# OPENAIRINTERFACE/openairinterface5g

Measured on AMD Instinct MI355X. Metric: ldpc_decoder_coded_throughput, higher is better.
Workload: dtype int8

## Files before the change

openairinterface5g_amd/csrc/ldpc_dec_fast_block.h:

```cpp
#ifndef LDPC_DEC_FAST_BLOCK_H
#define LDPC_DEC_FAST_BLOCK_H
#include <hip/hip_runtime.h>
#include "ldpc_kernels.h"
#include "ldpc_dec_fast_core.h"

typedef const ldpc_dec_job LDPC_CONST_AS *ldpc_job_ptr_t;


#ifndef LDPC_DEC_LLR_ARGS
#define LDPC_DEC_LLR_ARGS 1
#endif
#ifndef LDPC_DEC_LLR_TOGETHER
#define LDPC_DEC_LLR_TOGETHER 1
#endif
#ifndef LDPC_DEC_WARM
#define LDPC_DEC_WARM 0
#endif

#ifndef LDPC_MUTE_ITEMS
#define LDPC_MUTE_ITEMS 1
#endif
#define LDPC_EAGER_MAX_BAD_LANES 96
#define LDPC_TIMING_SLOTS 28
#ifndef LDPC_SYN_SKIP
#define LDPC_SYN_SKIP 1
#endif

#define LDPC_Q_TICKET(w) ((int)((uint32_t)(w) & 0xffffu))
#define LDPC_Q_BAD(w) ((int)((uint32_t)(w) >> 16))

__device__ __forceinline__ int ldpc_draw(int *counter, int lane)
{
  int t = 0;
  if (lane == 0)
    t = atomicAdd(counter, 1);
  return LDPC_UNIFORM(t);
}

__device__ __forceinline__ int ldpc_draw_count(int *counter, int lane, uint32_t syn)
{
  const int cnt = (int)__popcll(__ballot(syn != 0));
  int t = 0;
  if (lane == 0)
    t = atomicAdd(counter, 1 + (cnt << 16));
  return LDPC_UNIFORM(t);
}

__device__ __forceinline__ int ldpc_draw_issue(int *counter, int lane)
{
  int t = 0;
  if (lane == 0)
    t = __hip_atomic_fetch_add(counter, 1, __ATOMIC_RELAXED, __HIP_MEMORY_SCOPE_WORKGROUP);
  return t;
}

__device__ __forceinline__ int ldpc_desc_n_app(ldpc_code_ptr_t code, int zq) { return code->ncore * zq; }
__device__ __forceinline__ int ldpc_desc_n_ext(ldpc_code_ptr_t code, int zq) { return code->f_ext_global ? 0 : (code->ncols - code->ncore) * zq; }

#if defined(__HIP_DEVICE_COMPILE__)
#define LDPC_STAMP_BEHIND_S(x) asm volatile("" ::"s"(x) : "memory")
#define LDPC_STAMP_BEHIND_V(x) asm volatile("" ::"v"(x) : "memory")
#define LDPC_STAMP_BEHIND_ALL() __builtin_amdgcn_s_waitcnt(0)
#else
#define LDPC_STAMP_BEHIND_S(x) do { volatile uint32_t ldpc_keep_ = (uint32_t)(x); (void)ldpc_keep_; } while (0)
#define LDPC_STAMP_BEHIND_V(x) LDPC_STAMP_BEHIND_S(x)
#define LDPC_STAMP_BEHIND_ALL() ((void)0)
#endif

__device__ __forceinline__ void ldpc_fast_tables_to_lds(uint8_t *fsm, ldpc_code_ptr_t code, int tid, int nt)
{
  const uint32_t lds0 = ldpc_lds_addr(fsm);
  const int ext_global = code->f_ext_global, ncore = code->ncore, nedges = code->nedges, Z = code->Z;
  uint32_t *etbl = reinterpret_cast<uint32_t *>(fsm + code->f_lds_etbl);
  uint32_t *ctbl = reinterpret_cast<uint32_t *>(fsm + code->f_lds_ctbl);
  uint32_t *rowtbl = reinterpret_cast<uint32_t *>(fsm + code->f_lds_rowtbl);
  uint32_t *coltbl = reinterpret_cast<uint32_t *>(fsm + code->f_lds_coltbl);
  for (int i = tid; i < nedges; i += nt)
    etbl[i] = code->f_etbl[i] + ((ext_global && code->e_col[i] >= ncore) ? 0u : lds0);
  for (int i = tid; i < 2 * code->f_n_ctbl; i += nt)
    ctbl[i] = code->f_ctbl[i] + ((i & 1) ? lds0 : 0u);
  for (int i = tid; i < code->nrows; i += nt)
    rowtbl[i] = code->f_rowtbl[i];
  for (int i = tid; i < ncore; i += nt)
    coltbl[i] = code->f_coltbl[i];
  for (int i = tid; i < (Z + 4) >> 2; i += nt)
    reinterpret_cast<uint32_t *>(fsm + code->f_lds_zero)[i] = 0u;
}

__device__ __forceinline__ bool ldpc_fast_item_is_mute(const ldpc_fast_lds &L, int e0, int deg, int j)
{
  const uint32_t info = L.etbl[e0 + deg - 1];
  const uint32_t lw = L.ext_global ? (*reinterpret_cast<const uint32_t *>(L.gllr + info + 4u * (uint32_t)j) ^ 0x80808080u)
                                   : ldpc_lds_ld32(L.base, info + 4u * (uint32_t)j);
  return lw == 0x80808080u;
}
__device__ __forceinline__ void ldpc_fast_item_zero_messages(const ldpc_fast_lds &L, int e0, int deg, int j, int Z, int rstride)
{
  uint8_t *rrow = L.r + e0 * rstride + 4 * j;
  uint8_t *rpad = rrow + (j == 0 ? Z : 0);
  for (int k = 0; k < deg; k++) {
    *reinterpret_cast<uint32_t *>(rrow + k * rstride) = 0x80808080u;
    *reinterpret_cast<uint32_t *>(rpad + k * rstride) = 0x80808080u;
  }
}

template <class IO, int ZC = 0>
__device__ __forceinline__ int ldpc_dec_fast_block(uint8_t *fsm, ldpc_code_ptr_t code, const IO &io)
{
  const int Z = ZC ? ZC : code->Z, zq = ZC ? ZC / 4 : code->f_zq, rstride = ZC ? ZC + 4 : code->f_rstride,
            astride = ZC ? 2 * ZC : code->f_astride;
  const uint32_t zq_magic = ZC ? (uint32_t)((0x100000000ULL + (unsigned long long)(ZC ? ZC / 4 : 1) - 1) / (unsigned long long)(ZC ? ZC / 4 : 1))
                               : code->f_zq_magic;
  const uint32_t z_magic = 0xffffffffu / (uint32_t)Z + 1u;
  ldpc_fast_lds L;
  L.base = fsm;
  L.r = fsm + code->f_lds_r;
  L.app = fsm + code->f_lds_app;
  L.ext = fsm + code->f_lds_ext;
  uint32_t *etbl = reinterpret_cast<uint32_t *>(fsm + code->f_lds_etbl);
  uint32_t *ctbl = reinterpret_cast<uint32_t *>(fsm + code->f_lds_ctbl);
  uint32_t *rowtbl = reinterpret_cast<uint32_t *>(fsm + code->f_lds_rowtbl);
  uint32_t *coltbl = reinterpret_cast<uint32_t *>(fsm + code->f_lds_coltbl);
  L.etbl = etbl; L.ctbl = ctbl; L.rowtbl = rowtbl; L.coltbl = coltbl;
  int *flags = reinterpret_cast<int *>(fsm + code->f_lds_misc);
  const int tid = io.tid(), nt = blockDim.x, lane = tid & 63;
  const int ncore = code->ncore, num_llr = code->num_llr, ncz = ncore * Z;
  const uint32_t *__restrict__ src32 = io.src32();
  const uint32_t *__restrict__ srcp = io.src32_prologue();
  uint32_t *stage = io.stage_core();

  const int ext_global = code->f_ext_global;
  L.gllr = reinterpret_cast<const uint8_t *>(src32);
  L.ext_global = ext_global;
  const int n_app = io.n_app(code, zq), n_ext = io.n_ext(code, zq);
  uint32_t va[4], ve[4];
  if (!stage) {
#pragma unroll
    for (int k = 0; k < 4; k++) {
      const int ia = tid + k * nt;
#if LDPC_DEC_LLR_TOGETHER
      va[k] = io.ld_llr(srcp + (ia < n_app ? ia : 0));
      ve[k] = io.ld_llr(srcp + (ia < n_ext ? n_app + ia : 0));
#else
      va[k] = ia < n_app ? io.ld_llr(srcp + ia) : 0u;
      ve[k] = ia < n_ext ? io.ld_llr(srcp + n_app + ia) : 0u;
#endif
    }
  }
  if constexpr (IO::pass_stamps) {
    if (tid == 0) {
      LDPC_STAMP_BEHIND_S(ncore + num_llr + ext_global);
      io.stamps()[42] = (uint32_t)wall_clock64();
    }
    if (tid == nt - 64) {
      LDPC_STAMP_BEHIND_V(va[0]);
      io.stamps()[43] = (uint32_t)wall_clock64();
    }
  }
  const bool have_tables = io.tables_resident();
  if (!have_tables)
    ldpc_fast_tables_to_lds(fsm, code, tid, nt);
  if constexpr (IO::pass_stamps) {
    if (tid == 0) {
      LDPC_STAMP_BEHIND_ALL();
      io.stamps()[44] = (uint32_t)wall_clock64();
    }
  }
  if (stage) {
#pragma unroll
    for (int k = 0; k < 4; k++) {
      const int ia = tid + k * nt;
      va[k] = ia < n_app ? io.ld_llr(srcp + ia) : 0u;
      ve[k] = ia < n_ext ? io.ld_llr(srcp + n_app + ia) : 0u;
    }
  }
  if (tid < 16)
    flags[tid] = 0;
  uint32_t *e32 = reinterpret_cast<uint32_t *>(L.ext);
#pragma unroll
  for (int k = 0; k < 4; k++) {
    const int i = tid + k * nt;
    if (i < n_app) {
      const int c = (int)ldpc_umulhi((uint32_t)i, zq_magic), j = i - c * zq;
      const uint32_t w = va[k] ^ 0x80808080u;
      uint32_t *dst = reinterpret_cast<uint32_t *>(L.app + c * astride) + j;
      dst[0] = w;
      dst[zq] = w;
      if (stage)
        stage[i] = va[k];
    }
    if (i < n_ext)
      e32[i] = ve[k] ^ 0x80808080u;
  }
  for (int i = tid + 4 * nt; i < n_app; i += nt) {
    const int c = (int)ldpc_umulhi((uint32_t)i, zq_magic), j = i - c * zq;
    const uint32_t v = io.ld_llr(srcp + i), w = v ^ 0x80808080u;
    uint32_t *dst = reinterpret_cast<uint32_t *>(L.app + c * astride) + j;
    dst[0] = w;
    dst[zq] = w;
    if (stage)
      stage[i] = v;
  }
  for (int i = tid + 4 * nt; i < n_ext; i += nt)
    e32[i] = io.ld_llr(srcp + n_app + i) ^ 0x80808080u;
  __syncthreads();
  if (io.stamps() && tid == 0)
    io.stamps()[0] = (uint32_t)wall_clock64();

  const int max_pass = io.max_pass();
  int n_iter = max_pass;
  const int n_cn_tasks = code->f_n_cn_tasks, n_bn_tickets = code->f_n_bn_tickets, n_bn_tasks = code->f_n_bn_tasks,
            bn_group = code->f_bn_group;
  int cn_ticket = 0;
  bool mute_check = false;
  if constexpr (!IO::syndrome && IO::mute_items)
    mute_check = io.mute_check();
  (void)mute_check;
#ifdef LDPC_TIMING
  long long *tlog = reinterpret_cast<long long *>(io.out()) + (tid >> 6) * 2 * LDPC_TIMING_SLOTS;
  int tlog_n = 0;
  const long long t_kernel0 = clock64();
#define LDPC_TLOG_BEGIN() const long long tl0_ = clock64()
#define LDPC_TLOG_END(phase, deg) \
  do { \
    if (blockIdx.x == 0 && p == 2 && lane == 0 && tlog_n < LDPC_TIMING_SLOTS) { \
      tlog[2 * tlog_n] = ((tl0_ - t_kernel0) << 20) | ((long long)(phase) << 8) | (long long)(deg); \
      tlog[2 * tlog_n + 1] = clock64() - t_kernel0; \
      tlog_n++; \
    } \
  } while (0)
#define LDPC_TSTAMP(id) \
  do { \
    LDPC_TLOG_BEGIN(); \
    LDPC_TLOG_END(3, id); \
  } while (0)
#else
#define LDPC_TLOG_BEGIN() do { } while (0)
#define LDPC_TLOG_END(phase, deg) do { } while (0)
#define LDPC_TSTAMP(id) do { } while (0)
#endif
  const int fair = io.fair_turns();
  int prio_slot = 0;
  if (fair)
    prio_slot = (int)(__builtin_amdgcn_s_getreg((3 << 11) | 4) & 15u) / fair;
  for (int p = 1; p <= max_pass; ++p) {
    uint32_t tsyn = 0;
    bool skip = false;
    if (fair) {
      if ((p + prio_slot) & 1)
        __builtin_amdgcn_s_setprio(1);
      else
        __builtin_amdgcn_s_setprio(0);
    }
    if constexpr (IO::warm_next && LDPC_DEC_WARM != 0) {
      if (p == 2 && tid >= nt - 64) {
        if (const uint32_t *nx = io.warm_row()) {
          const int n_lines = (num_llr + 127) >> 7, last = (num_llr >> 2) - 1;
          uint32_t got = 0;
          for (int t0 = lane; t0 <= n_lines; t0 += 256) {
#pragma unroll
            for (int k = 0; k < 4; k++) {
              const int i = 32 * (t0 + 64 * k);
              got ^= nx[i < last ? i : last];
            }
          }
          LDPC_STAMP_BEHIND_V(got);
        }
      }
    }
    const uint32_t ab_word = (io.has_abort() && tid == 0 && p >= 2) ? io.abort_load() : 0u;
    int tb_ab = 0;
    if (io.has_abort() && tid == 0 && p >= 2 && io.tb_abort())
      tb_ab = __hip_atomic_load(io.tb_abort(), __ATOMIC_RELAXED, __HIP_MEMORY_SCOPE_AGENT);
    int *const pq = &flags[8 + (p & 1)];
#ifdef LDPC_ABLATE_CN
    int task = cn_ticket;
    if (IO::syndrome && lane == 0)
      atomicAdd(pq, 64 << 16);
#else
    if (p == 1)
      cn_ticket = LDPC_Q_TICKET(ldpc_draw(pq, lane));
    int task = cn_ticket;
    auto next_task = [&]() -> int {
      if constexpr (IO::syndrome) {
        const int w = ldpc_draw_count(pq, lane, tsyn);
        skip = LDPC_SYN_SKIP && LDPC_Q_BAD(w) > LDPC_EAGER_MAX_BAD_LANES;
        if constexpr (IO::pass_stamps) {
          if (skip && LDPC_Q_TICKET(w) < n_cn_tasks && lane == 0)
            atomicAdd(&flags[7], 1);
        }
        return LDPC_Q_TICKET(w);
      } else {
        return LDPC_Q_TICKET(ldpc_draw(pq, lane));
      }
    };
    for (; task < n_cn_tasks; task = next_task()) {
      LDPC_TLOG_BEGIN();
      tsyn = 0;
      bool with_syn = false;
      if constexpr (IO::syndrome)
        with_syn = p >= 2 && !skip;
      const int deg_f = code->f_cn_task[task][0], ext = code->f_cn_task[task][1];
      const int item = code->f_cn_task[task][2] + lane;
      const int gstart = code->f_cn_task[task][3], gend = code->f_cn_task[task][4], srow0 = code->f_cn_task[task][5];
      const int deg = deg_f & 0xff;
      if (deg_f & 0x100) {
        if (item < gend) {
          const int item_b = item + 64 < gend ? item + 64 : item;
          const int gia = item - gstart, gib = item_b - gstart;
          const int riga = (int)ldpc_umulhi((uint32_t)gia, zq_magic), ja = gia - riga * zq;
          const int rigb = (int)ldpc_umulhi((uint32_t)gib, zq_magic), jb = gib - rigb * zq;
          const uint32_t reca = rowtbl[srow0 + riga], recb = rowtbl[srow0 + rigb];
          const int e0a = (int)(reca & 0x1ffu), e0b = (int)(recb & 0x1ffu);
          uint32_t mb = 0;
          bool mute = false;
          if constexpr (!IO::syndrome && IO::mute_items)
            mute = mute_check && ldpc_fast_item_is_mute(L, e0a, deg, ja) && ldpc_fast_item_is_mute(L, e0b, deg, jb);
          if (mute) {
            if (p == 1) {
              ldpc_fast_item_zero_messages(L, e0a, deg, ja, Z, rstride);
              ldpc_fast_item_zero_messages(L, e0b, deg, jb, Z, rstride);
            }
          } else if (p == 1)
            (void)ldpc_fast_cn2_dispatch<true, false>(deg, L, e0a, ja, e0b, jb, Z, rstride, mb);
          else if (with_syn) {
            if constexpr (IO::syndrome) {
              const uint32_t ma = ldpc_fast_cn2_dispatch<false, true>(deg, L, e0a, ja, e0b, jb, Z, rstride, mb);
              const int valida = (int)(reca >> 16) - 4 * ja, validb = (int)(recb >> 16) - 4 * jb;
              tsyn = (ma & ldpc_fast_valid_lanes(valida)) | (mb & ldpc_fast_valid_lanes(validb));
            }
          } else
            (void)ldpc_fast_cn2_dispatch<false, false>(deg, L, e0a, ja, e0b, jb, Z, rstride, mb);
        }
      } else if (item < gend) {
        const bool pair = deg == 19 && code->f_pair19;
        const int gi = pair ? (item - gstart) >> 1 : item - gstart, half = (item - gstart) & 1;
        const int rig = (int)ldpc_umulhi((uint32_t)gi, zq_magic), j = gi - rig * zq;
        const uint32_t rowrec = rowtbl[srow0 + rig];
        const int e0 = (int)(rowrec & 0x1ffu);
        (void)half;
#if !defined(__HIP_DEVICE_COMPILE__)
        if (pair && half)
          continue;
#endif
        bool mute = false;
        if constexpr (!IO::syndrome && IO::mute_items)
          mute = mute_check && ext && ldpc_fast_item_is_mute(L, e0, deg, j);
        if (mute) {
          if (p == 1)
            ldpc_fast_item_zero_messages(L, e0, deg, j, Z, rstride);
        } else if (p == 1) {
#if defined(__HIP_DEVICE_COMPILE__)
          if (pair)
            (void)ldpc_fast_cn19_pair<true, false>(L, e0, j, Z, rstride, half);
          else
#endif
            (void)ldpc_fast_cn_dispatch<true, false>(deg, ext, L, e0, j, Z, rstride);
        } else if (with_syn) {
          if constexpr (IO::syndrome) {
            uint32_t m;
#if defined(__HIP_DEVICE_COMPILE__)
            if (pair)
              m = ldpc_fast_cn19_pair<false, true>(L, e0, j, Z, rstride, half);
            else
#endif
              m = ldpc_fast_cn_dispatch<false, true>(deg, ext, L, e0, j, Z, rstride);
            const int valid = (int)(rowrec >> 16) - 4 * j;
            tsyn = m & ldpc_fast_valid_lanes(valid);
          }
        } else {
#if defined(__HIP_DEVICE_COMPILE__)
          if (pair)
            (void)ldpc_fast_cn19_pair<false, false>(L, e0, j, Z, rstride, half);
          else
#endif
            (void)ldpc_fast_cn_dispatch<false, false>(deg, ext, L, e0, j, Z, rstride);
        }
      }
      LDPC_TLOG_END(0, deg);
    }
#endif
    const int bn_ticket = task - n_cn_tasks;
    if (tid == 0) {
      flags[2] = 0;
      flags[8 + ((p + 1) & 1)] = 0;
      if (tb_ab)
        flags[3] = 1;
      if (p >= 2 && io.abort_is(ab_word))
        flags[3] = 1;
    }
    __syncthreads();
    const int bad_prev = LDPC_Q_BAD(__hip_atomic_load(pq, __ATOMIC_RELAXED, __HIP_MEMORY_SCOPE_WORKGROUP));
    if constexpr (IO::pass_stamps) {
      if (tid == 0 && p <= 9) {
        io.stamps()[2 * p] = (uint32_t)wall_clock64();
        io.stamps()[22 + p] = (uint32_t)bad_prev;
        io.stamps()[32 + p] = (uint32_t)flags[7];
      }
      if (tid == 0)
        flags[7] = 0;
    }
    if (io.has_abort() && flags[3]) {
      n_iter = max_pass + 1;
      break;
    }
    if (!io.use_crc() && p >= 3 && bad_prev == 0) {
      n_iter = p - 1;
      break;
    }
#ifndef LDPC_ABLATE_BN
    if constexpr (IO::bn_tickets) {
    for (int ticket = bn_ticket, nxt = 0; ticket < n_bn_tickets; ticket = LDPC_Q_TICKET(LDPC_UNIFORM(nxt)) - n_cn_tasks) {
      LDPC_TLOG_BEGIN();
      const int item0 = code->f_bn_rec[ticket][0] + lane, end = code->f_bn_rec[ticket][1];
      const int maxdeg = code->f_bn_rec[ticket][2], cnt = code->f_bn_rec[ticket][3];
      if (cnt == 1) {
        if (item0 < end) {
          const int sc = (int)ldpc_umulhi((uint32_t)item0, zq_magic), j = item0 - sc * zq;
          const uint32_t colrec = coltbl[sc];
          const uint32_t lw = src32[(int)(colrec & 0xffu) * zq + j];
          uint32_t ae = 0, at = 0;
          ldpc_fast_bn_gather(L, colrec, maxdeg, j, Z, 0, ae, at);
          nxt = ldpc_draw_issue(pq, lane);
          ldpc_fast_bn_finish(L, (int)(colrec & 0xffu), (int)((colrec >> 8) & 0xffu), j, Z, astride, lw, ae, at, 0);
        } else {
          nxt = ldpc_draw_issue(pq, lane);
        }
      } else {
        uint32_t rec[LDPC_F_BN_GROUP], lw[LDPC_F_BN_GROUP];
        int jj[LDPC_F_BN_GROUP];
        bool live[LDPC_F_BN_GROUP];
#pragma unroll
        for (int g = 0; g < LDPC_F_BN_GROUP; g++) {
          const int item = item0 + 64 * g;
          live[g] = g < cnt && item < end;
          const int it = live[g] ? item : end - 1;
          const int sc = (int)ldpc_umulhi((uint32_t)it, zq_magic);
          jj[g] = it - sc * zq;
          rec[g] = coltbl[sc];
          lw[g] = src32[(int)(rec[g] & 0xffu) * zq + jj[g]];
        }
        ldpc_fast_bn_multi<LDPC_F_BN_GROUP>(L, rec, jj, lw, live, maxdeg, Z, astride);
        nxt = ldpc_draw_issue(pq, lane);
      }
      LDPC_TLOG_END(1, maxdeg);
    }
    } else {
    for (int ticket = bn_ticket; ticket * bn_group < n_bn_tasks; ticket = LDPC_Q_TICKET(ldpc_draw(pq, lane)) - n_cn_tasks) {
      for (int task = ticket * bn_group; task < (ticket + 1) * bn_group && task < n_bn_tasks; task++) {
        LDPC_TLOG_BEGIN();
        const int item = code->f_bn_task[task][0] + lane, end = code->f_bn_task[task][1];
        const int maxdeg = code->f_bn_task[task][2];
        if (item < end) {
          const int sc = (int)ldpc_umulhi((uint32_t)item, zq_magic), j = item - sc * zq;
          const uint32_t colrec = coltbl[sc];
          const uint32_t lw = src32[(int)(colrec & 0xffu) * zq + j];
          ldpc_fast_bn(L, colrec, maxdeg, j, Z, astride, lw);
        }
        LDPC_TLOG_END(1, maxdeg);
      }
    }
    }
#endif
    cn_ticket = LDPC_Q_TICKET(ldpc_draw(&flags[8 + ((p + 1) & 1)], lane));
    __syncthreads();
    if constexpr (IO::pass_stamps) {
      if (tid == 0 && p <= 9)
        io.stamps()[2 * p + 1] = (uint32_t)wall_clock64();
    }
    if (io.eager_check() && !io.use_crc() && p >= 2 && p < max_pass && bad_prev <= LDPC_EAGER_MAX_BAD_LANES) {
      if constexpr (IO::pass_stamps) {
        if (tid == 0)
          io.stamps()[20] |= 1u << p;
      }
      uint32_t esyn = 0;
      const int n_items = code->nrows * zq;
      for (int item = tid; item < n_items; item += nt) {
        const int sr = (int)ldpc_umulhi((uint32_t)item, zq_magic), j = item - sr * zq;
        const uint32_t rowrec = rowtbl[sr];
        const int e0 = (int)(rowrec & 0x1ffu), deg = (int)((rowrec >> 9) & 0x1fu), ext = (int)((rowrec >> 14) & 1u);
        const int valid = (int)(rowrec >> 16) - 4 * j;
        const uint32_t m = ldpc_fast_pc(L, deg, ext, e0, j, rstride);
        esyn |= m & ldpc_fast_valid_lanes(valid);
      }
      if (__any(esyn != 0) && lane == 0)
        flags[6] = 1;
      __syncthreads();
      const int bad = flags[6];
      __syncthreads();
      if (tid == 0)
        flags[6] = 0;
      if (!bad) {
        n_iter = p;
        break;
      }
      __syncthreads();
    }
    if (io.use_crc() && p >= 3) {
      uint32_t x = 0;
      const int crcE = io.crcE();
      const uint32_t *crc_pow = io.crc_pow();
#pragma unroll 1
      for (int i = 4 * tid; i < crcE; i += 4 * nt) {
        const int c = (int)ldpc_umulhi((uint32_t)i, z_magic), u = i - c * Z;
        const uint32_t nb = ~*reinterpret_cast<const uint32_t *>(L.app + c * astride + u);
        const uint4 pw = *reinterpret_cast<const uint4 *>(crc_pow + (crcE - 4 - i));
        const uint32_t p3 = pw.w, p2 = pw.z, p1 = pw.y, p0 = pw.x;
        x ^= (p3 & (0u - ((nb >> 7) & 1u))) ^ (p2 & (0u - ((nb >> 15) & 1u))) ^ (p1 & (0u - ((nb >> 23) & 1u))) ^
             (p0 & (0u - (nb >> 31)));
      }
      for (int off = 32; off; off >>= 1)
        x ^= __shfl_xor(x, off);
      if (lane == 0 && x)
        atomicXor(reinterpret_cast<unsigned int *>(&flags[2]), x);
      __syncthreads();
      const int rem = flags[2];
      __syncthreads();
      if (rem == 0) {
        n_iter = p;
        break;
      }
    }
  }
  if (io.stamps() && tid == 0)
    io.stamps()[1] = (uint32_t)wall_clock64();
  if (io.tb_abort() && n_iter == max_pass && tid == 0)
    __hip_atomic_store(io.tb_abort(), 1, __ATOMIC_RELAXED, __HIP_MEMORY_SCOPE_AGENT);

#ifdef LDPC_TIMING
  if (blockIdx.x == 0)
    return n_iter;
#endif
  auto bits_word = [&](int w) -> uint32_t {
    uint32_t word = 0;
#pragma unroll
    for (int q = 0; q < 8; q++) {
      const int b = 32 * w + 4 * q;
      if (b < ncz) {
        const int c = (int)ldpc_umulhi((uint32_t)b, z_magic), u = b - c * Z;
        const uint32_t nb = ~*reinterpret_cast<const uint32_t *>(L.app + c * astride + u);
        const uint32_t nib = (((nb >> 7) & 1u) << 3) | (((nb >> 15) & 1u) << 2) | (((nb >> 23) & 1u) << 1) | (nb >> 31);
        word |= nib << (8 * (q >> 1) + ((q & 1) ? 0 : 4));
      }
    }
    return word;
  };
  auto bytes_word = [&](int w) -> uint32_t {
    const int b = 4 * w;
    if (b >= ncz)
      return 0u;
    const int c = (int)ldpc_umulhi((uint32_t)b, z_magic), u = b - c * Z;
    const uint32_t nb = ~*reinterpret_cast<const uint32_t *>(L.app + c * astride + u);
    return (nb >> 7) & 0x01010101u;
  };
  if constexpr (IO::tb_epilogue) {
    if (io.tb_fused()) {
      io.tb_finish(n_iter, bits_word, flags);
      return n_iter;
    }
  }
  if ((!io.use_crc() || n_iter >= 3) && n_iter <= max_pass) {
    const uint32_t tag = io.out_tag();
    const int nwords = io.out_mode() == 0 ? (num_llr + 31) >> 5 : num_llr >> 2;
    if (tag) {
      uint4 *o16 = reinterpret_cast<uint4 *>(io.out());
      for (int c = tid; 3 * c < nwords; c += nt) {
        uint32_t w3[3];
#pragma unroll
        for (int q = 0; q < 3; q++) {
          const int w = 3 * c + q;
          w3[q] = w < nwords ? (io.out_mode() == 0 ? bits_word(w) : bytes_word(w)) : 0u;
        }
        io.put16(o16 + c, w3[0], w3[1], w3[2], tag);
      }
    } else if (io.out_mode() == 0) {
      uint32_t *o = reinterpret_cast<uint32_t *>(io.out());
      for (int w = tid; w < nwords; w += nt)
        o[w] = bits_word(w);
    } else {
      int8_t *o = io.out();
      for (int i = tid; i < num_llr; i += nt)
        o[i] = (i < ncz) ? (int8_t)ldpc_fast_hd(L, i, Z, z_magic, astride) : (int8_t)0;
    }
  }
  return n_iter;
}
#endif
```

openairinterface5g_amd/csrc/ldpc_dec_fast_core.h:

```cpp
#ifndef LDPC_DEC_FAST_CORE_H
#define LDPC_DEC_FAST_CORE_H
#include "ldpc_dec_core.h"

#if !defined(__HIPCC__)
struct uint2 { uint32_t x, y; };
#endif
typedef short ldpc_v2i __attribute__((ext_vector_type(2)));
typedef unsigned short ldpc_v2u __attribute__((ext_vector_type(2)));

#if defined(__HIP_DEVICE_COMPILE__)
LDPC_HD uint32_t ldpc_perm(uint32_t s0, uint32_t s1, uint32_t sel) { return __builtin_amdgcn_perm(s0, s1, sel); }
LDPC_HD uint32_t ldpc_alignbyte(uint32_t hi, uint32_t lo, uint32_t sh) { return __builtin_amdgcn_alignbyte(hi, lo, sh); }
LDPC_HD uint32_t ldpc_umulhi(uint32_t a, uint32_t b) { return __umulhi(a, b); }
#else
LDPC_HD uint32_t ldpc_perm(uint32_t s0, uint32_t s1, uint32_t sel)
{
  const uint64_t src = ((uint64_t)s0 << 32) | s1;
  uint32_t r = 0;
  for (int i = 0; i < 4; i++) {
    const uint32_t s = (sel >> (8 * i)) & 0xff;
    const uint32_t b = s <= 7    ? (uint32_t)((src >> (8 * s)) & 0xff)
                       : s <= 11 ? (((src >> (16 * (s - 8) + 15)) & 1) ? 0xffu : 0u)
                                 : (s == 0x0c ? 0u : 0xffu);
    r |= b << (8 * i);
  }
  return r;
}
LDPC_HD uint32_t ldpc_alignbyte(uint32_t hi, uint32_t lo, uint32_t sh)
{
  return (uint32_t)(((((uint64_t)hi) << 32) | lo) >> (8 * (sh & 3)));
}
LDPC_HD uint32_t ldpc_umulhi(uint32_t a, uint32_t b) { return (uint32_t)(((uint64_t)a * b) >> 32); }
#endif

LDPC_HD ldpc_v2i ldpc_as_v2i(uint32_t x) { return __builtin_bit_cast(ldpc_v2i, x); }
LDPC_HD ldpc_v2u ldpc_as_v2u(uint32_t x) { return __builtin_bit_cast(ldpc_v2u, x); }
LDPC_HD uint32_t ldpc_u2u32(ldpc_v2u x) { return __builtin_bit_cast(uint32_t, x); }
LDPC_HD ldpc_v2u ldpc_splatu(unsigned v) { return (ldpc_v2u){(unsigned short)v, (unsigned short)v}; }
LDPC_HD ldpc_v2u ldpc_pminu(ldpc_v2u a, ldpc_v2u b) { return __builtin_elementwise_min(a, b); }
LDPC_HD ldpc_v2u ldpc_pmaxu(ldpc_v2u a, ldpc_v2u b) { return __builtin_elementwise_max(a, b); }
#define LDPC_KEY_NEUTRAL 0xfbffu
LDPC_HD ldpc_v2u ldpc_pmin3_keys(ldpc_v2u a, ldpc_v2u b, ldpc_v2u c)
{
#if defined(__HIP_DEVICE_COMPILE__)
  uint32_t r;
  asm("v_pk_maximum3_f16 %0, %1, %2, %3" : "=v"(r) : "v"(__builtin_bit_cast(uint32_t, a)), "v"(__builtin_bit_cast(uint32_t, b)),
      "v"(__builtin_bit_cast(uint32_t, c)));
  return __builtin_bit_cast(ldpc_v2u, r);
#else
  return __builtin_elementwise_min(__builtin_elementwise_min(a, b), c);
#endif
}
LDPC_HD uint32_t ldpc_psub_sm(uint32_t a, uint32_t r)
{
#if defined(__HIP_DEVICE_COMPILE__)
  typedef _Float16 ldpc_v2h __attribute__((ext_vector_type(2)));
  const uint32_t d = __builtin_bit_cast(uint32_t, __builtin_bit_cast(ldpc_v2h, a) - __builtin_bit_cast(ldpc_v2h, r));
  return d;
#else
  uint32_t d = 0;
  for (int h = 0; h < 32; h += 16) {
    const uint32_t x = (a >> h) & 0xffffu, y = (r >> h) & 0xffffu;
    d |= (x < y ? 0x8000u | (y - x) : x - y) << h;
  }
  return d;
#endif
}
LDPC_HD ldpc_v2u ldpc_sm_key(uint32_t d) { return __builtin_bit_cast(ldpc_v2u, d | 0x80008000u); }
LDPC_HD uint32_t ldpc_unpack_even(uint32_t w) { return w & 0x00ff00ffu; }
LDPC_HD uint32_t ldpc_unpack_odd(uint32_t w) { return ldpc_perm(0u, w, 0x0c030c01u); }
LDPC_HD uint32_t ldpc_as_u32(ldpc_v2i x) { return __builtin_bit_cast(uint32_t, x); }
LDPC_HD ldpc_v2i ldpc_splat(int v) { return (ldpc_v2i){(short)v, (short)v}; }
LDPC_HD ldpc_v2i ldpc_pmin(ldpc_v2i a, ldpc_v2i b) { return __builtin_elementwise_min(a, b); }
LDPC_HD ldpc_v2i ldpc_pmax(ldpc_v2i a, ldpc_v2i b) { return __builtin_elementwise_max(a, b); }
LDPC_HD ldpc_v2i ldpc_unpack_lo(uint32_t w) { return ldpc_as_v2i(ldpc_perm(0u, w, 0x0c010c00u)); }
LDPC_HD ldpc_v2i ldpc_unpack_hi(uint32_t w) { return ldpc_as_v2i(ldpc_perm(0u, w, 0x0c030c02u)); }
LDPC_HD uint32_t ldpc_pack4(ldpc_v2i lo, ldpc_v2i hi) { return ldpc_perm(ldpc_as_u32(hi), ldpc_as_u32(lo), 0x06040200u); }

struct ldpc_fast_lds {
  uint8_t *base;
  uint8_t *r;
  uint8_t *app;
  uint8_t *ext;
  const uint32_t *etbl, *ctbl, *rowtbl, *coltbl;
  const uint8_t *gllr;
  int ext_global;
};

#if defined(__HIP_DEVICE_COMPILE__)
LDPC_HD uint32_t ldpc_lds_addr(const uint8_t *p) { return (uint32_t)(uintptr_t)(const __attribute__((address_space(3))) uint8_t *)p; }
LDPC_HD uint32_t ldpc_lds_ld32(const uint8_t *, uint32_t a) { return *(const __attribute__((address_space(3))) uint32_t *)a; }
#else
LDPC_HD uint32_t ldpc_lds_addr(const uint8_t *) { return 0u; }
LDPC_HD uint32_t ldpc_lds_ld32(const uint8_t *base, uint32_t a) { return *reinterpret_cast<const uint32_t *>(base + a); }
#endif
LDPC_HD uint32_t ldpc_window_al(const uint8_t *base, uint32_t a, uint32_t sh)
{
  return ldpc_alignbyte(ldpc_lds_ld32(base, a + 4u), ldpc_lds_ld32(base, a), sh);
}
LDPC_HD uint32_t ldpc_window(const uint8_t *base, uint32_t off) { return ldpc_window_al(base, off & ~3u, off); }

#define LDPC_SEL_EO 0x07030501u
#define LDPC_SEL_SIGNS 0x0b090a08u
template <uint32_t SEL = 0x07050301u>
LDPC_HD uint32_t ldpc_fast_odd_lanes(uint32_t parw, bool ext, uint32_t extl, uint32_t exth, int D)
{
  uint32_t np = parw >> 7;
  if (ext)
    np ^= ldpc_perm(exth, extl, SEL);
  if (D & 1)
    np = ~np;
  return np & 0x01010101u;
}
LDPC_HD uint32_t ldpc_fast_valid_lanes(int valid) { return valid > 0 ? 0x01010101u : 0u; }
LDPC_HD uint32_t ldpc_fast_cn_sign_acc(uint32_t sx4, uint32_t s4_prev, uint32_t s4_k, int k, int D)
{
  if (k & 1) {
#if defined(__HIP_DEVICE_COMPILE__)
    return __builtin_amdgcn_bitop3_b32(sx4, s4_prev, s4_k, 0x96);
#else
    return sx4 ^ s4_prev ^ s4_k;
#endif
  }
  return k == D - 1 ? sx4 ^ s4_k : sx4;
}
LDPC_HD uint32_t ldpc_fast_cn_out_bytes(uint32_t o4, uint32_t sx4, uint32_t s4)
{
#if defined(__HIP_DEVICE_COMPILE__)
  return __builtin_amdgcn_bitop3_b32(o4, sx4, s4, 0x96) + __builtin_amdgcn_bitop3_b32(sx4, s4, 0x01010101u, 0x28);
#else
  const uint32_t x4 = sx4 ^ s4;
  return (o4 ^ x4) + (x4 & 0x01010101u);
#endif
}

template <bool IS_EXT, bool P1 = false>
LDPC_HD void ldpc_fast_cn_edge(const ldpc_fast_lds &L, uint32_t info, int t, uint32_t rw, bool first, uint32_t &de, uint32_t &dod,
                               uint32_t &parw, uint32_t &exte, uint32_t &exto)
{
  if (IS_EXT) {
    const uint32_t lw = L.ext_global ? (*reinterpret_cast<const uint32_t *>(L.gllr + info + (uint32_t)t) ^ 0x80808080u)
                                     : ldpc_lds_ld32(L.base, info + (uint32_t)t);
    const uint32_t ae = ldpc_unpack_even(lw), ao = ldpc_unpack_odd(lw);
    if (first) {
      exte = ae + (P1 ? 0x00800080u : ldpc_unpack_even(rw));
      exto = ao + (P1 ? 0x00800080u : ldpc_unpack_odd(rw));
    }
    de = ldpc_psub_sm(ae, 0x00800080u);
    dod = ldpc_psub_sm(ao, 0x00800080u);
  } else {
    const uint32_t aw = ldpc_window(L.base, info + (uint32_t)t);
    if (first)
      parw ^= aw;
    if (P1) {
      de = ldpc_psub_sm(ldpc_unpack_even(aw), 0x00800080u);
      dod = ldpc_psub_sm(ldpc_unpack_odd(aw), 0x00800080u);
    } else {
      de = ldpc_psub_sm(ldpc_unpack_even(aw), ldpc_unpack_even(rw));
      dod = ldpc_psub_sm(ldpc_unpack_odd(aw), ldpc_unpack_odd(rw));
    }
  }
}

template <int D, bool EXT, int MODE, bool P1 = false, bool SYN = true>
LDPC_HD uint32_t ldpc_fast_cn(const ldpc_fast_lds &L, int e0, int j, int Z, int rstride, int boff_r = 0, int boff_a = 0)
{
  const int t = 4 * j + boff_r, ta = 4 * j + boff_a;
  constexpr bool KEEP = MODE == 0;
  uint32_t d_lo[MODE <= 1 ? D : 1], d_hi[MODE <= 1 ? D : 1], g_lo[KEEP ? D : 1], g_hi[KEEP ? D : 1];
  ldpc_v2u m1l = ldpc_splatu(0xffff), m2l = m1l, m1h = m1l, m2h = m1l;
  uint32_t sxl = 0, sxh = 0, parw = 0, extl = 0, exth = 0;
  uint8_t *rrow = L.r + e0 * rstride + t;
  uint8_t *rpad = rrow + (j == 0 ? Z : 0);
#pragma unroll
  for (int k = 0; k < D; k++) {
    const uint32_t info = L.etbl[e0 + k];
    const uint32_t rw = (P1 || (!SYN && EXT && k == D - 1)) ? 0u : *reinterpret_cast<const uint32_t *>(rrow + k * rstride);
    uint32_t dl, dh;
    if (EXT && k == D - 1)
      ldpc_fast_cn_edge<true, P1>(L, info, t, rw, SYN, dl, dh, parw, extl, exth);
    else
      ldpc_fast_cn_edge<false, P1>(L, info, ta, rw, SYN, dl, dh, parw, extl, exth);
    if (MODE <= 1) {
      d_lo[k] = dl;
      d_hi[k] = dh;
    }
    const ldpc_v2u ml = ldpc_sm_key(dl);
    const ldpc_v2u mh = ldpc_sm_key(dh);
    if (KEEP) {
      g_lo[k] = ldpc_u2u32(ml);
      g_hi[k] = ldpc_u2u32(mh);
    }
    sxl ^= dl;
    sxh ^= dh;
    m2l = ldpc_pminu(m2l, ldpc_pmaxu(m1l, ml));
    m1l = ldpc_pminu(m1l, ml);
    m2h = ldpc_pminu(m2h, ldpc_pmaxu(m1h, mh));
    m1h = ldpc_pminu(m1h, mh);
  }
  const ldpc_v2u cap = ldpc_splatu(0x8000 + 127);
  m1l = ldpc_pminu(m1l, cap); m2l = ldpc_pminu(m2l, cap);
  m1h = ldpc_pminu(m1h, cap); m2h = ldpc_pminu(m2h, cap);
  const uint32_t sl = (ldpc_u2u32(m1l) - 0x80008000u) + ldpc_u2u32(m2l), sh = (ldpc_u2u32(m1h) - 0x80008000u) + ldpc_u2u32(m2h);
  const uint32_t sx4 = ldpc_perm(sxh, sxl, LDPC_SEL_SIGNS) ^ 0x80808080u;
#pragma unroll
  for (int k = 0; k < D; k++) {
    uint32_t dl, dh;
    if (MODE <= 1) {
      dl = d_lo[k];
      dh = d_hi[k];
    } else {
      const uint32_t info = L.etbl[e0 + k];
      const uint32_t rw = (P1 || (EXT && k == D - 1)) ? 0u : *reinterpret_cast<const uint32_t *>(rrow + k * rstride);
      if (EXT && k == D - 1)
        ldpc_fast_cn_edge<true, P1>(L, info, t, rw, false, dl, dh, parw, extl, exth);
      else
        ldpc_fast_cn_edge<false, P1>(L, info, ta, rw, false, dl, dh, parw, extl, exth);
    }
    const ldpc_v2u ml = KEEP ? ldpc_as_v2u(g_lo[k]) : ldpc_sm_key(dl);
    const ldpc_v2u mh = KEEP ? ldpc_as_v2u(g_hi[k]) : ldpc_sm_key(dh);
    const uint32_t ol = sl - ldpc_u2u32(ldpc_pminu(ml, m2l)), oh = sh - ldpc_u2u32(ldpc_pminu(mh, m2h));
    const uint32_t o4 = ldpc_perm(oh, ol, 0x06020400u);
    const uint32_t w = ldpc_fast_cn_out_bytes(o4, sx4, ldpc_perm(dh, dl, LDPC_SEL_SIGNS));
    *reinterpret_cast<uint32_t *>(rrow + k * rstride) = w;
    *reinterpret_cast<uint32_t *>(rpad + k * rstride) = w;
  }
  return SYN ? ldpc_fast_odd_lanes<LDPC_SEL_EO>(parw, EXT, extl, exth, D) : 0u;
}

template <int D, bool EXT, bool P1 = false, bool SYN = true>
LDPC_HD uint32_t ldpc_fast_cn_ps(const ldpc_fast_lds &L, int e0, int j, int Z, int rstride, int boff_r = 0, int boff_a = 0)
{
  const int t = 4 * j + boff_r, ta = 4 * j + boff_a;
  constexpr int NP = D / 2;
  uint32_t m_lo[D], m_hi[D], p_lo[NP], p_hi[NP], s4[D];
  const ldpc_v2u cap = ldpc_splatu(0x8000 + 127);
  uint32_t sx4 = 0, parw = 0, extl = 0, exth = 0;
  uint8_t *rrow = L.r + e0 * rstride + t;
  uint8_t *rpad = rrow + (j == 0 ? Z : 0);
#pragma unroll
  for (int k = 0; k < D; k++) {
    const uint32_t info = L.etbl[e0 + k];
    const uint32_t rw = (P1 || (!SYN && EXT && k == D - 1)) ? 0u : *reinterpret_cast<const uint32_t *>(rrow + k * rstride);
    uint32_t dl, dh;
    if (EXT && k == D - 1)
      ldpc_fast_cn_edge<true, P1>(L, info, t, rw, SYN, dl, dh, parw, extl, exth);
    else
      ldpc_fast_cn_edge<false, P1>(L, info, ta, rw, SYN, dl, dh, parw, extl, exth);
    const ldpc_v2u ml = ldpc_sm_key(dl);
    const ldpc_v2u mh = ldpc_sm_key(dh);
    m_lo[k] = ldpc_u2u32(ml);
    m_hi[k] = ldpc_u2u32(mh);
    s4[k] = ldpc_perm(dh, dl, LDPC_SEL_SIGNS);
    sx4 = ldpc_fast_cn_sign_acc(sx4, k ? s4[k - 1] : 0u, s4[k], k, D);
    if ((k & 1) && k < D - 1) {
      const int i = k / 2;
      p_lo[i] = ldpc_u2u32(ldpc_pmin3_keys(i ? ldpc_as_v2u(p_lo[i - 1]) : cap, ldpc_as_v2u(m_lo[k - 1]), ml));
      p_hi[i] = ldpc_u2u32(ldpc_pmin3_keys(i ? ldpc_as_v2u(p_hi[i - 1]) : cap, ldpc_as_v2u(m_hi[k - 1]), mh));
    }
  }
  sx4 ^= 0x80808080u;
  auto put = [&](int k, ldpc_v2u ol, ldpc_v2u oh) {
    const uint32_t o4 = ldpc_perm(ldpc_u2u32(oh), ldpc_u2u32(ol), 0x06020400u);
    const uint32_t w = ldpc_fast_cn_out_bytes(o4, sx4, s4[k]);
    *reinterpret_cast<uint32_t *>(rrow + k * rstride) = w;
    *reinterpret_cast<uint32_t *>(rpad + k * rstride) = w;
  };
  ldpc_v2u sl = cap, sh = cap;
  if (D & 1) {
    put(D - 1, ldpc_as_v2u(p_lo[NP - 1]), ldpc_as_v2u(p_hi[NP - 1]));
    sl = ldpc_as_v2u(m_lo[D - 1]);
    sh = ldpc_as_v2u(m_hi[D - 1]);
  }
#pragma unroll
  for (int i = NP - 1; i >= 0; i--) {
    const int k0 = 2 * i, k1 = 2 * i + 1;
    const ldpc_v2u pvl = i ? ldpc_as_v2u(p_lo[i - 1]) : cap, pvh = i ? ldpc_as_v2u(p_hi[i - 1]) : cap;
    const ldpc_v2u a0l = ldpc_as_v2u(m_lo[k0]), a0h = ldpc_as_v2u(m_hi[k0]), a1l = ldpc_as_v2u(m_lo[k1]), a1h = ldpc_as_v2u(m_hi[k1]);
    const bool last = !(D & 1) && i == NP - 1;
    put(k0, last ? ldpc_pminu(pvl, a1l) : ldpc_pmin3_keys(pvl, a1l, sl), last ? ldpc_pminu(pvh, a1h) : ldpc_pmin3_keys(pvh, a1h, sh));
    put(k1, last ? ldpc_pminu(pvl, a0l) : ldpc_pmin3_keys(pvl, a0l, sl), last ? ldpc_pminu(pvh, a0h) : ldpc_pmin3_keys(pvh, a0h, sh));
    if (i > 0) {
      sl = last ? ldpc_pminu(a0l, a1l) : ldpc_pmin3_keys(sl, a0l, a1l);
      sh = last ? ldpc_pminu(a0h, a1h) : ldpc_pmin3_keys(sh, a0h, a1h);
    }
  }
  return SYN ? ldpc_fast_odd_lanes<LDPC_SEL_EO>(parw, EXT, extl, exth, D) : 0u;
}

template <int D, bool EXT, bool P1 = false, bool SYN = true>
LDPC_HD uint32_t ldpc_fast_cn_ps2(const ldpc_fast_lds &L, int e0a, int ja, int e0b, int jb, int Z, int rstride, uint32_t &mask_b)
{
  constexpr int N = 2, NP = D / 2;
  const int e0[N] = {e0a, e0b}, t[N] = {4 * ja, 4 * jb};
  uint32_t m_lo[N][D], m_hi[N][D], p_lo[N][NP > 0 ? NP : 1], p_hi[N][NP > 0 ? NP : 1], s4[N][D];
  const ldpc_v2u cap = ldpc_splatu(0x8000 + 127);
  uint32_t sx4[N] = {0, 0}, parw[N] = {0, 0}, extl[N] = {0, 0}, exth[N] = {0, 0};
  uint8_t *rrow[N], *rpad[N];
#pragma unroll
  for (int n = 0; n < N; n++) {
    rrow[n] = L.r + e0[n] * rstride + t[n];
    rpad[n] = rrow[n] + (t[n] == 0 ? Z : 0);
  }
#pragma unroll
  for (int k = 0; k < D; k++) {
    uint32_t info[N], rw[N];
#pragma unroll
    for (int n = 0; n < N; n++) {
      info[n] = L.etbl[e0[n] + k];
      rw[n] = (P1 || (!SYN && EXT && k == D - 1)) ? 0u : *reinterpret_cast<const uint32_t *>(rrow[n] + k * rstride);
    }
#pragma unroll
    for (int n = 0; n < N; n++) {
      uint32_t dl, dh;
      if (EXT && k == D - 1)
        ldpc_fast_cn_edge<true, P1>(L, info[n], t[n], rw[n], SYN, dl, dh, parw[n], extl[n], exth[n]);
      else
        ldpc_fast_cn_edge<false, P1>(L, info[n], t[n], rw[n], SYN, dl, dh, parw[n], extl[n], exth[n]);
      const ldpc_v2u ml = ldpc_sm_key(dl);
      const ldpc_v2u mh = ldpc_sm_key(dh);
      m_lo[n][k] = ldpc_u2u32(ml);
      m_hi[n][k] = ldpc_u2u32(mh);
      s4[n][k] = ldpc_perm(dh, dl, LDPC_SEL_SIGNS);
      sx4[n] = ldpc_fast_cn_sign_acc(sx4[n], k ? s4[n][k - 1] : 0u, s4[n][k], k, D);
      if ((k & 1) && k < D - 1) {
        const int i = k / 2;
        p_lo[n][i] = ldpc_u2u32(ldpc_pmin3_keys(i ? ldpc_as_v2u(p_lo[n][i - 1]) : cap, ldpc_as_v2u(m_lo[n][k - 1]), ml));
        p_hi[n][i] = ldpc_u2u32(ldpc_pmin3_keys(i ? ldpc_as_v2u(p_hi[n][i - 1]) : cap, ldpc_as_v2u(m_hi[n][k - 1]), mh));
      }
    }
  }
  sx4[0] ^= 0x80808080u;
  sx4[1] ^= 0x80808080u;
  auto put = [&](int n, int k, ldpc_v2u ol, ldpc_v2u oh) {
    const uint32_t o4 = ldpc_perm(ldpc_u2u32(oh), ldpc_u2u32(ol), 0x06020400u);
    const uint32_t w = ldpc_fast_cn_out_bytes(o4, sx4[n], s4[n][k]);
    *reinterpret_cast<uint32_t *>(rrow[n] + k * rstride) = w;
    *reinterpret_cast<uint32_t *>(rpad[n] + k * rstride) = w;
  };
  ldpc_v2u sl[N] = {cap, cap}, sh[N] = {cap, cap};
  if (D & 1) {
#pragma unroll
    for (int n = 0; n < N; n++) {
      put(n, D - 1, NP ? ldpc_as_v2u(p_lo[n][NP - 1]) : cap, NP ? ldpc_as_v2u(p_hi[n][NP - 1]) : cap);
      sl[n] = ldpc_as_v2u(m_lo[n][D - 1]);
      sh[n] = ldpc_as_v2u(m_hi[n][D - 1]);
    }
  }
#pragma unroll
  for (int i = NP - 1; i >= 0; i--) {
    const int k0 = 2 * i, k1 = 2 * i + 1;
    const bool last = !(D & 1) && i == NP - 1;
#pragma unroll
    for (int n = 0; n < N; n++) {
      const ldpc_v2u pvl = i ? ldpc_as_v2u(p_lo[n][i - 1]) : cap, pvh = i ? ldpc_as_v2u(p_hi[n][i - 1]) : cap;
      const ldpc_v2u a0l = ldpc_as_v2u(m_lo[n][k0]), a0h = ldpc_as_v2u(m_hi[n][k0]), a1l = ldpc_as_v2u(m_lo[n][k1]), a1h = ldpc_as_v2u(m_hi[n][k1]);
      put(n, k0, last ? ldpc_pminu(pvl, a1l) : ldpc_pmin3_keys(pvl, a1l, sl[n]), last ? ldpc_pminu(pvh, a1h) : ldpc_pmin3_keys(pvh, a1h, sh[n]));
      put(n, k1, last ? ldpc_pminu(pvl, a0l) : ldpc_pmin3_keys(pvl, a0l, sl[n]), last ? ldpc_pminu(pvh, a0h) : ldpc_pmin3_keys(pvh, a0h, sh[n]));
      if (i > 0) {
        sl[n] = last ? ldpc_pminu(a0l, a1l) : ldpc_pmin3_keys(sl[n], a0l, a1l);
        sh[n] = last ? ldpc_pminu(a0h, a1h) : ldpc_pmin3_keys(sh[n], a0h, a1h);
      }
    }
  }
  uint32_t out[N];
#pragma unroll
  for (int n = 0; n < N; n++) {
    out[n] = SYN ? ldpc_fast_odd_lanes<LDPC_SEL_EO>(parw[n], EXT, extl[n], exth[n], D) : 0u;
  }
  mask_b = out[1];
  return out[0];
}
#if defined(__HIP_DEVICE_COMPILE__) && defined(LDPC_CN2_NOINLINE)
#define LDPC_CN2_ATTR __device__ __attribute__((noinline))
#else
#define LDPC_CN2_ATTR LDPC_HD
#endif
template <bool P1 = false, bool SYN = true>
LDPC_CN2_ATTR uint32_t ldpc_fast_cn2_dispatch(int deg, const ldpc_fast_lds &L, int e0a, int ja, int e0b, int jb, int Z, int rstride, uint32_t &mask_b)
{
  switch (deg) {
    case 3: return ldpc_fast_cn_ps2<3, true, P1, SYN>(L, e0a, ja, e0b, jb, Z, rstride, mask_b);
    case 4: return ldpc_fast_cn_ps2<4, true, P1, SYN>(L, e0a, ja, e0b, jb, Z, rstride, mask_b);
    default: return ldpc_fast_cn_ps2<5, true, P1, SYN>(L, e0a, ja, e0b, jb, Z, rstride, mask_b);
  }
}

#if defined(__HIP_DEVICE_COMPILE__)
__device__ __forceinline__ uint32_t ldpc_swap_pair(uint32_t v) { return (uint32_t)__builtin_amdgcn_update_dpp(0, (int)v, 0xB1 , 0xf, 0xf, false); }
template <bool P1, bool SYN = true>
__device__ __forceinline__ uint32_t ldpc_fast_cn19_pair(const ldpc_fast_lds &L, int e0, int j, int Z, int rstride, int half)
{
  constexpr int N = 10, NP = N / 2;
  const int t = 4 * j;
  const int ebase = e0 + (half ? 10 : 0);
  uint32_t m_lo[N], m_hi[N], p_lo[NP], p_hi[NP], s4[N];
  const ldpc_v2u cap = ldpc_splatu(0x8000 + 127);
  uint32_t sx4 = 0, parw = 0, extl = 0, exth = 0;
  uint8_t *rrow = L.r + ebase * rstride + t;
  uint8_t *rpad = rrow + (j == 0 ? Z : 0);
#pragma unroll
  for (int k = 0; k < N; k++) {
    const bool live = k < N - 1 || !half;
    const int kk = live ? k : N - 2;
    const uint32_t info = L.etbl[ebase + kk];
    const uint32_t rw = P1 ? 0u : *reinterpret_cast<const uint32_t *>(rrow + kk * rstride);
    uint32_t dl, dh, pw = 0;
    ldpc_fast_cn_edge<false, P1>(L, info, t, rw, SYN, dl, dh, pw, extl, exth);
    ldpc_v2u ml = ldpc_sm_key(dl);
    ldpc_v2u mh = ldpc_sm_key(dh);
    uint32_t sg = ldpc_perm(dh, dl, LDPC_SEL_SIGNS);
    if (!live) {
      ml = mh = ldpc_splatu(LDPC_KEY_NEUTRAL);
      sg = 0u;
      pw = 0u;
    }
    m_lo[k] = ldpc_u2u32(ml); m_hi[k] = ldpc_u2u32(mh);
    s4[k] = sg;
    sx4 = ldpc_fast_cn_sign_acc(sx4, k ? s4[k - 1] : 0u, sg, k, N);
    if (SYN)
      parw ^= pw;
    if (k & 1) {
      const int i = k / 2;
      p_lo[i] = ldpc_u2u32(ldpc_pmin3_keys(i ? ldpc_as_v2u(p_lo[i - 1]) : cap, ldpc_as_v2u(m_lo[k - 1]), ml));
      p_hi[i] = ldpc_u2u32(ldpc_pmin3_keys(i ? ldpc_as_v2u(p_hi[i - 1]) : cap, ldpc_as_v2u(m_hi[k - 1]), mh));
    }
  }
  ldpc_v2u sl = ldpc_as_v2u(ldpc_swap_pair(p_lo[NP - 1])), sh = ldpc_as_v2u(ldpc_swap_pair(p_hi[NP - 1]));
  sx4 ^= ldpc_swap_pair(sx4);
  if (SYN)
    parw ^= ldpc_swap_pair(parw);
  sx4 ^= 0x80808080u;
#pragma unroll
  for (int i = NP - 1; i >= 0; i--) {
    const ldpc_v2u pvl = i ? ldpc_as_v2u(p_lo[i - 1]) : cap, pvh = i ? ldpc_as_v2u(p_hi[i - 1]) : cap;
#pragma unroll
    for (int q = 0; q < 2; q++) {
      const int k = 2 * i + q, ko = 2 * i + 1 - q;
      const bool live = k < N - 1 || !half;
      const ldpc_v2u ol = ldpc_pmin3_keys(pvl, ldpc_as_v2u(m_lo[ko]), sl), oh = ldpc_pmin3_keys(pvh, ldpc_as_v2u(m_hi[ko]), sh);
      const uint32_t o4 = ldpc_perm(ldpc_u2u32(oh), ldpc_u2u32(ol), 0x06020400u);
      const uint32_t w = ldpc_fast_cn_out_bytes(o4, sx4, s4[k]);
      if (live) {
        *reinterpret_cast<uint32_t *>(rrow + k * rstride) = w;
        *reinterpret_cast<uint32_t *>(rpad + k * rstride) = w;
      }
    }
    if (i > 0) {
      sl = ldpc_pmin3_keys(sl, ldpc_as_v2u(m_lo[2 * i]), ldpc_as_v2u(m_lo[2 * i + 1]));
      sh = ldpc_pmin3_keys(sh, ldpc_as_v2u(m_hi[2 * i]), ldpc_as_v2u(m_hi[2 * i + 1]));
    }
  }
  return SYN ? ldpc_fast_odd_lanes(parw, false, 0u, 0u, 19) : 0u;
}
#endif

LDPC_HD uint32_t ldpc_fast_pc(const ldpc_fast_lds &L, int D, int ext, int e0, int j, int rstride)
{
  const int t = 4 * j;
  uint32_t parw = 0;
  const int ncore_edges = ext ? D - 1 : D;
  int k = 0;
  for (; k + 4 <= ncore_edges; k += 4) {
    uint32_t info[4], lo[4], hi[4];
#pragma unroll
    for (int i = 0; i < 4; i++)
      info[i] = L.etbl[e0 + k + i] + (uint32_t)t;
#pragma unroll
    for (int i = 0; i < 4; i++) {
      lo[i] = ldpc_lds_ld32(L.base, info[i] & ~3u);
      hi[i] = ldpc_lds_ld32(L.base, (info[i] & ~3u) + 4u);
    }
#pragma unroll
    for (int i = 0; i < 4; i++)
      parw ^= ldpc_alignbyte(hi[i], lo[i], info[i]);
  }
  for (; k < ncore_edges; k++)
    parw ^= ldpc_window(L.base, L.etbl[e0 + k] + (uint32_t)t);
  uint32_t extl = 0, exth = 0;
  if (ext) {
    const uint32_t info = L.etbl[e0 + D - 1];
    const uint32_t lw = L.ext_global ? (*reinterpret_cast<const uint32_t *>(L.gllr + info + (uint32_t)t) ^ 0x80808080u)
                                     : ldpc_lds_ld32(L.base, info + (uint32_t)t);
    const uint32_t rw = *reinterpret_cast<const uint32_t *>(L.r + (e0 + D - 1) * rstride + t);
    extl = ldpc_perm(0x80808080u, lw, 0x05010400u) + ldpc_perm(0u, rw, 0x0c010c00u);
    exth = ldpc_perm(0x80808080u, lw, 0x05030402u) + ldpc_perm(0u, rw, 0x0c030c02u);
  }
  return ldpc_fast_odd_lanes(parw, ext != 0, extl, exth, D);
}

#ifndef LDPC_F_MODE_D19
#define LDPC_F_MODE_D19 2
#endif
template <bool P1 = false, bool SYN = true>
LDPC_HD uint32_t ldpc_fast_cn_dispatch(int deg, int ext, const ldpc_fast_lds &L, int e0, int j, int Z, int rstride, int boff_r = 0,
                                       int boff_a = 0)
{
  if (!ext) {
    switch (deg) {
      case 19: return ldpc_fast_cn<19, false, LDPC_F_MODE_D19, P1, SYN>(L, e0, j, Z, rstride, boff_r, boff_a);
      case 10: return ldpc_fast_cn_ps<10, false, P1, SYN>(L, e0, j, Z, rstride, boff_r, boff_a);
      default: return ldpc_fast_cn_ps<8, false, P1, SYN>(L, e0, j, Z, rstride, boff_r, boff_a);
    }
  }
  switch (deg) {
    case 3: return ldpc_fast_cn_ps<3, true, P1, SYN>(L, e0, j, Z, rstride, boff_r, boff_a);
    case 4: return ldpc_fast_cn_ps<4, true, P1, SYN>(L, e0, j, Z, rstride, boff_r, boff_a);
    case 5: return ldpc_fast_cn_ps<5, true, P1, SYN>(L, e0, j, Z, rstride, boff_r, boff_a);
    case 6: return ldpc_fast_cn_ps<6, true, P1, SYN>(L, e0, j, Z, rstride, boff_r, boff_a);
    case 7: return ldpc_fast_cn_ps<7, true, P1, SYN>(L, e0, j, Z, rstride, boff_r, boff_a);
    case 8: return ldpc_fast_cn_ps<8, true, P1, SYN>(L, e0, j, Z, rstride, boff_r, boff_a);
    case 9: return ldpc_fast_cn_ps<9, true, P1, SYN>(L, e0, j, Z, rstride, boff_r, boff_a);
    default: return ldpc_fast_cn_ps<10, true, P1, SYN>(L, e0, j, Z, rstride, boff_r, boff_a);
  }
}

LDPC_HD void ldpc_fast_bn_acc(uint32_t w, uint32_t &ae, uint32_t &at)
{
  ae += w & 0x00ff00ffu;
  at += w >> 8;
}
LDPC_HD uint32_t ldpc_fast_bn_odd_sums(uint32_t ae, uint32_t at) { return at - ((ae >> 16) << 8); }

LDPC_HD void ldpc_fast_bn_gather_from(const ldpc_fast_lds &L, int first, int maxdeg, int j, int Z, int boff_r, uint32_t &ae,
                                      uint32_t &at)
{
  const int u = 4 * j;
  const uint2 *tbl = reinterpret_cast<const uint2 *>(L.ctbl) + first;
  int k = 0;
  uint2 ce[4];
  if (maxdeg >= 4) {
#pragma unroll
    for (int i = 0; i < 4; i++)
      ce[i] = tbl[i];
  }
  for (; k + 4 <= maxdeg; k += 4) {
    uint32_t lo[4], hi[4], ph[4];
#pragma unroll
    for (int i = 0; i < 4; i++) {
      const uint32_t q = (uint32_t)u + ce[i].x;
      const uint32_t p = q < q - (uint32_t)Z ? q : q - (uint32_t)Z;
      const uint32_t a = ce[i].y + p + (uint32_t)boff_r;
      lo[i] = ldpc_lds_ld32(L.base, a);
      hi[i] = ldpc_lds_ld32(L.base, a + 4u);
      ph[i] = q;
    }
    if (k + 8 <= maxdeg) {
#pragma unroll
      for (int i = 0; i < 4; i++)
        ce[i] = tbl[k + 4 + i];
    }
#pragma unroll
    for (int i = 0; i < 4; i++)
      ldpc_fast_bn_acc(ldpc_alignbyte(hi[i], lo[i], ph[i]), ae, at);
  }
  for (; k < maxdeg; k++) {
    const uint2 c1 = tbl[k];
    const uint32_t q = (uint32_t)u + c1.x;
    const uint32_t p = q < q - (uint32_t)Z ? q : q - (uint32_t)Z;
    ldpc_fast_bn_acc(ldpc_window_al(L.base, c1.y + p + (uint32_t)boff_r, q), ae, at);
  }
}
LDPC_HD void ldpc_fast_bn_gather(const ldpc_fast_lds &L, uint32_t colrec, int maxdeg, int j, int Z, int boff_r, uint32_t &ae,
                                 uint32_t &at)
{
  ldpc_fast_bn_gather_from(L, (int)(colrec >> 16), maxdeg, j, Z, boff_r, ae, at);
}
LDPC_HD void ldpc_fast_bn_finish(const ldpc_fast_lds &L, int c, int deg, int j, int Z, int astride, uint32_t llr_word, uint32_t ae,
                                 uint32_t at, int boff_a)
{
  const int u = 4 * j;
  ldpc_fast_bn_acc(llr_word ^ 0x80808080u, ae, at);
  const uint32_t acc_e = ae, acc_o = ldpc_fast_bn_odd_sums(ae, at);
#if defined(__HIP_DEVICE_COMPILE__) && !defined(LDPC_NO_SAT_PK)
  const ldpc_v2i bias = ldpc_splat(deg * 128);
  uint32_t se, so;
  asm("v_sat_pk_u8_i16 %0, %1" : "=v"(se) : "v"(ldpc_as_u32(ldpc_as_v2i(acc_e) - bias)));
  asm("v_sat_pk_u8_i16 %0, %1" : "=v"(so) : "v"(ldpc_as_u32(ldpc_as_v2i(acc_o) - bias)));
  const uint32_t w = ldpc_perm(so, se, 0x05010400u);
#else
  const ldpc_v2i bias = ldpc_splat((deg + 1) * 128), lo = ldpc_splat(-128), hi = ldpc_splat(127), b128 = ldpc_splat(128);
  const ldpc_v2i ve = ldpc_pmin(ldpc_pmax(ldpc_as_v2i(acc_e) - bias, lo), hi) + b128;
  const ldpc_v2i vo = ldpc_pmin(ldpc_pmax(ldpc_as_v2i(acc_o) - bias, lo), hi) + b128;
  const uint32_t w = ldpc_perm(ldpc_as_u32(vo), ldpc_as_u32(ve), 0x06020400u);
#endif
  uint32_t *dst = reinterpret_cast<uint32_t *>(L.app + c * astride + u + boff_a);
  dst[0] = w;
  *reinterpret_cast<uint32_t *>(L.app + c * astride + u + boff_a + Z) = w;
}
LDPC_HD void ldpc_fast_bn(const ldpc_fast_lds &L, uint32_t colrec, int maxdeg, int j, int Z, int astride,
                          uint32_t llr_word, int boff_r = 0, int boff_a = 0)
{
  uint32_t ae = 0, at = 0;
  ldpc_fast_bn_gather(L, colrec, maxdeg, j, Z, boff_r, ae, at);
  ldpc_fast_bn_finish(L, (int)(colrec & 0xffu), (int)((colrec >> 8) & 0xffu), j, Z, astride, llr_word, ae, at, boff_a);
}

template <int G>
LDPC_HD void ldpc_fast_bn_multi(const ldpc_fast_lds &L, const uint32_t (&rec)[G], const int (&jj)[G], const uint32_t (&lw)[G],
                                const bool (&live)[G], int md, int Z, int astride)
{
  uint32_t ae[G], at[G];
  const uint2 *tbl[G];
#pragma unroll
  for (int g = 0; g < G; g++) {
    ae[g] = at[g] = 0u;
    tbl[g] = reinterpret_cast<const uint2 *>(L.ctbl) + (int)(rec[g] >> 16);
  }
  for (int k = 0; k < md; k++) {
    uint2 ce[G];
    uint32_t lo[G], hi[G], ph[G];
#pragma unroll
    for (int g = 0; g < G; g++)
      ce[g] = tbl[g][k];
#pragma unroll
    for (int g = 0; g < G; g++) {
      const uint32_t q = 4u * (uint32_t)jj[g] + ce[g].x;
      const uint32_t p = q < q - (uint32_t)Z ? q : q - (uint32_t)Z;
      const uint32_t a = ce[g].y + p;
      lo[g] = ldpc_lds_ld32(L.base, a);
      hi[g] = ldpc_lds_ld32(L.base, a + 4u);
      ph[g] = q;
    }
#pragma unroll
    for (int g = 0; g < G; g++)
      ldpc_fast_bn_acc(ldpc_alignbyte(hi[g], lo[g], ph[g]), ae[g], at[g]);
  }
#pragma unroll
  for (int g = 0; g < G; g++)
    if (live[g])
      ldpc_fast_bn_finish(L, (int)(rec[g] & 0xffu), (int)((rec[g] >> 8) & 0xffu), jj[g], Z, astride, lw[g], ae[g], at[g], 0);
}

LDPC_HD int ldpc_fast_hd(const ldpc_fast_lds &L, int b, int Z, uint32_t zmagic, int astride)
{
  const int c = (int)ldpc_umulhi((uint32_t)b, zmagic), u = b - c * Z;
  return L.app[c * astride + u] < 128;
}
#endif
```

openairinterface5g_amd/csrc/ldpc_decoder_fast.hip:

```cpp
#include <hip/hip_runtime.h>
#include <cstdlib>
#include "ldpc_kernels.h"
#include "ldpc_dec_fast_block.h"
#include "ldpc_dec_fast_mblock.h"

template <bool JOBS, bool CRC = false, bool TRACE = false> struct ldpc_batch_io {
  const ldpc_dec_args &a;
  ldpc_job_ptr_t job;
  __device__ __forceinline__ const uint32_t *src32() const
  {
    return reinterpret_cast<const uint32_t *>(a.llr + (job ? (size_t)job->llr_off : (size_t)blockIdx.x * a.llr_stride));
  }
  __device__ __forceinline__ int8_t *out() const { return a.out + (job ? (size_t)job->out_off : (size_t)blockIdx.x * a.out_stride); }
  __device__ __forceinline__ int max_pass() const { return (job ? job->num_max_iter : a.num_max_iter) + 1; }
  __device__ __forceinline__ int use_crc() const { return CRC ? 1 : 0; }
  static constexpr bool syndrome = !CRC;
  __device__ __forceinline__ int crcE() const { return job ? job->E : a.E; }
  __device__ __forceinline__ const uint32_t *crc_pow() const { return job ? a.crc_pow_tbl[job->crc_type & 3] : a.crc_pow; }
  __device__ __forceinline__ int out_mode() const { return a.out_mode; }
  __device__ __forceinline__ int *tb_abort() const
  {
    return (job && a.tb_abort && job->abort_idx >= 0) ? a.tb_abort + job->abort_idx : nullptr;
  }
  __device__ __forceinline__ uint32_t *stamps() const
  {
    return TRACE ? reinterpret_cast<uint32_t *>(a.trace + (size_t)blockIdx.x * 32 + 5) : nullptr;
  }
  static constexpr bool pass_stamps = TRACE;
  __device__ __forceinline__ int fair_turns() const { return a.fair; }
  __device__ __forceinline__ int tid() const { return (int)threadIdx.x; }
  __device__ __forceinline__ bool eager_check() const { return !JOBS; }
  static constexpr bool mute_items = false;
  __device__ __forceinline__ bool mute_check() const { return false; }
  static constexpr bool bn_tickets = true;
  static constexpr bool tb_epilogue = false;
  __device__ __forceinline__ bool tables_resident() const { return false; }
  __device__ __forceinline__ uint32_t out_tag() const { return 0u; }
  __device__ __forceinline__ uint32_t abort_load() const { return 0u; }
  __device__ __forceinline__ bool abort_is(uint32_t) const { return false; }
  __device__ __forceinline__ bool has_abort() const { return JOBS; }
  __device__ __forceinline__ void put16(uint4 *p, uint32_t x, uint32_t y, uint32_t z, uint32_t t) const { *p = make_uint4(x, y, z, t); }
  __device__ __forceinline__ uint32_t ld_llr(const uint32_t *p) const { return *p; }
  __device__ __forceinline__ const uint32_t *src32_prologue() const { return src32(); }
  __device__ __forceinline__ uint32_t *stage_core() const { return nullptr; }
  __device__ __forceinline__ int n_app(ldpc_code_ptr_t code, int zq) const
  {
    return (!JOBS && LDPC_DEC_LLR_ARGS) ? (int)a.n_app : ldpc_desc_n_app(code, zq);
  }
  __device__ __forceinline__ int n_ext(ldpc_code_ptr_t code, int zq) const
  {
    return (!JOBS && LDPC_DEC_LLR_ARGS) ? (int)a.n_ext : ldpc_desc_n_ext(code, zq);
  }
  static constexpr bool warm_next = !JOBS;
  __device__ __forceinline__ const uint32_t *warm_row() const
  {
    const uint32_t nb = blockIdx.x + a.warm_ahead;
    if (a.warm_ahead == 0 || nb >= a.n_blocks)
      return nullptr;
    return reinterpret_cast<const uint32_t *>(a.llr + (size_t)nb * a.llr_stride);
  }
};

static void ldpc_fill_llr_extents(ldpc_dec_args &a, const ldpc_code_desc_t &hc)
{
  a.n_app = (uint32_t)(hc.ncore * hc.f_zq);
  a.n_ext = hc.f_ext_global ? 0u : (uint32_t)((hc.ncols - hc.ncore) * hc.f_zq);
}

template <bool JOBS, bool CRC = false, bool TRACE = false, int ZC = 0>
__global__ void __launch_bounds__(1024) ldpc_dec_fast_kernel(const ldpc_dec_args a)
{
  LDPC_DYNAMIC_LDS(uint8_t, fsm);
  const ldpc_job_ptr_t job = JOBS ? (ldpc_job_ptr_t)a.jobs + blockIdx.x : (ldpc_job_ptr_t) nullptr;
  ldpc_code_ptr_t code = (ldpc_code_ptr_t)(job ? job->code : a.code);
  const ldpc_batch_io<JOBS, CRC, TRACE> io{a, job};
  unsigned long long *tr = TRACE ? a.trace + (size_t)blockIdx.x * 32 : nullptr;
  if (TRACE && threadIdx.x == 0) {
    tr[0] = __builtin_amdgcn_s_getreg((31 << 11) | 4);
    tr[1] = __builtin_amdgcn_s_getreg((3 << 11) | 20);
    tr[2] = wall_clock64();
  }
  const int n_iter = ldpc_dec_fast_block<ldpc_batch_io<JOBS, CRC, TRACE>, ZC>(fsm, code, io);
  if (threadIdx.x == 0)
    a.n_iter[job ? (uint32_t)job->iter_idx : blockIdx.x] = n_iter;
  if (TRACE) {
    __syncthreads();
    if (threadIdx.x == 0) {
      tr[3] = wall_clock64();
      tr[4] = (unsigned long long)n_iter;
    }
  }
}

template <bool CRC>
__global__ void __launch_bounds__(1024) ldpc_dec_fast_pull_kernel(const ldpc_dec_args a)
{
  LDPC_DYNAMIC_LDS(uint8_t, fsm);
  ldpc_code_ptr_t code = (ldpc_code_ptr_t)a.code;
  const int nb = code->num_llr, tid = (int)threadIdx.x, nt = (int)blockDim.x;
  const uint8_t *src = reinterpret_cast<const uint8_t *>(a.pull) + (size_t)blockIdx.x * a.pull_stride;
  uint8_t *dst = reinterpret_cast<uint8_t *>(const_cast<int8_t *>(a.llr)) + (size_t)blockIdx.x * a.llr_stride;
  if (a.pull_stagger_ticks && blockIdx.x < a.pull_first_round) {
    const long long until = (long long)wall_clock64() + (long long)(blockIdx.x >> 6) * (long long)a.pull_stagger_ticks;
    while ((long long)wall_clock64() < until)
      __builtin_amdgcn_s_sleep(32);
  }
  if ((((uintptr_t)src | (uintptr_t)dst) & 15) == 0) {
    const uint4 *s16 = reinterpret_cast<const uint4 *>(src);
    uint4 *d16 = reinterpret_cast<uint4 *>(dst);
    const int n16 = nb >> 4;
    for (int i = tid; i < n16; i += 4 * nt) {
      const int last = n16 - 1;
      const int i1 = i + nt, i2 = i + 2 * nt, i3 = i + 3 * nt;
      const uint4 v0 = s16[i], v1 = s16[i1 < last ? i1 : last], v2 = s16[i2 < last ? i2 : last], v3 = s16[i3 < last ? i3 : last];
      d16[i] = v0;
      if (i1 < n16) d16[i1] = v1;
      if (i2 < n16) d16[i2] = v2;
      if (i3 < n16) d16[i3] = v3;
    }
    const int rest = (nb & 15) >> 2;
    if (tid < rest)
      reinterpret_cast<uint32_t *>(dst)[4 * n16 + tid] = reinterpret_cast<const uint32_t *>(src)[4 * n16 + tid];
  } else {
    const uint32_t *s4 = reinterpret_cast<const uint32_t *>(src);
    uint32_t *d4 = reinterpret_cast<uint32_t *>(dst);
    const int n4 = nb >> 2;
    for (int i = tid; i < n4; i += 4 * nt) {
      const int last = n4 - 1;
      const int i1 = i + nt, i2 = i + 2 * nt, i3 = i + 3 * nt;
      const uint32_t v0 = s4[i], v1 = s4[i1 < last ? i1 : last], v2 = s4[i2 < last ? i2 : last], v3 = s4[i3 < last ? i3 : last];
      d4[i] = v0;
      if (i1 < n4) d4[i1] = v1;
      if (i2 < n4) d4[i2] = v2;
      if (i3 < n4) d4[i3] = v3;
    }
  }
  __builtin_amdgcn_fence(__ATOMIC_RELEASE, "workgroup");
  __syncthreads();
  __builtin_amdgcn_fence(__ATOMIC_ACQUIRE, "workgroup");
  const ldpc_batch_io<false, CRC> io{a, (ldpc_job_ptr_t) nullptr};
  const int n_iter = ldpc_dec_fast_block(fsm, code, io);
  if (threadIdx.x == 0)
    a.n_iter[blockIdx.x] = n_iter;
}

template <int SUB, bool CRC>
__global__ void __launch_bounds__(1024) ldpc_dec_fast_multi_kernel(const ldpc_dec_args a)
{
  LDPC_DYNAMIC_LDS(uint8_t, fsm);
  ldpc_code_ptr_t code = (ldpc_code_ptr_t)a.code;
  const uint32_t per_wg = (uint32_t)code->f_mb * SUB;
  const uint32_t first = blockIdx.x * per_wg;
  const uint32_t left = a.n_blocks - first;
  const ldpc_mb_io<false> io{a, first, (ldpc_job_ptr_t) nullptr, a.num_max_iter, a.E, a.crc_pow};
  ldpc_dec_fast_mblock<SUB, false, CRC>(fsm, code, io, left < per_wg ? (int)left : (int)per_wg);
}
template <int SUB, bool CRC>
__global__ void __launch_bounds__(1024) ldpc_dec_fast_multi_jobs_kernel(const ldpc_dec_args a)
{
  LDPC_DYNAMIC_LDS(uint8_t, fsm);
  typedef const ldpc_dec_mgroup LDPC_CONST_AS *grp_ptr_t;
  const grp_ptr_t gr = (grp_ptr_t)a.mgroups + blockIdx.x;
  ldpc_code_ptr_t code = (ldpc_code_ptr_t)gr->code;
  const ldpc_mb_io<true> io{a, gr->first_job, (ldpc_job_ptr_t)a.jobs + gr->first_job, gr->num_max_iter, gr->E, a.crc_pow_tbl[gr->crc_type & 3]};
  ldpc_dec_fast_mblock<SUB, true, CRC>(fsm, code, io, (int)gr->n_valid);
}

bool ldpc_fast_zc_enabled(int zc)
{
  static const bool on = !(getenv("NRLDPC_HIP_ZC") && atoi(getenv("NRLDPC_HIP_ZC")) == 0);
  if (!on)
    return false;
  switch (zc) {
#define X(z) case z:
    LDPC_FAST_ZC_LIST(X)
#undef X
      return LDPC_FAST_ZC != 0;
    default:
      return false;
  }
}

template <bool JOBS, bool CRC>
static bool ldpc_launch_zc(int zc, uint32_t n_blocks, int n_threads, int lds_bytes, hipStream_t stream, const ldpc_dec_args &a)
{
  switch (zc) {
#define X(z) \
  case z: \
    hipLaunchKernelGGL((ldpc_dec_fast_kernel<JOBS, CRC, false, z>), dim3(n_blocks), dim3(n_threads), lds_bytes, stream, a); \
    return true;
    LDPC_FAST_ZC_LIST(X)
#undef X
    default:
      return false;
  }
}

hipError_t ldpc_fast_kernel_init(void)
{
  const void *k[] = {reinterpret_cast<const void *>(ldpc_dec_fast_kernel<false, false, true>),
                     reinterpret_cast<const void *>(ldpc_dec_fast_kernel<false>), reinterpret_cast<const void *>(ldpc_dec_fast_kernel<true>),
                     reinterpret_cast<const void *>(ldpc_dec_fast_kernel<true, true>), reinterpret_cast<const void *>(ldpc_dec_fast_kernel<false, true>),
#define X(z) \
                     reinterpret_cast<const void *>(ldpc_dec_fast_kernel<false, false, false, z>), \
                     reinterpret_cast<const void *>(ldpc_dec_fast_kernel<false, true, false, z>), \
                     reinterpret_cast<const void *>(ldpc_dec_fast_kernel<true, true, false, z>), \
                     reinterpret_cast<const void *>(ldpc_dec_fast_kernel<true, false, false, z>),
                     LDPC_FAST_ZC_LIST(X)
#undef X
                     reinterpret_cast<const void *>(ldpc_dec_fast_pull_kernel<false>), reinterpret_cast<const void *>(ldpc_dec_fast_pull_kernel<true>),
                     reinterpret_cast<const void *>(ldpc_dec_fast_multi_kernel<1, false>), reinterpret_cast<const void *>(ldpc_dec_fast_multi_kernel<1, true>),
                     reinterpret_cast<const void *>(ldpc_dec_fast_multi_kernel<4, false>), reinterpret_cast<const void *>(ldpc_dec_fast_multi_kernel<4, true>),
                     reinterpret_cast<const void *>(ldpc_dec_fast_multi_jobs_kernel<1, false>), reinterpret_cast<const void *>(ldpc_dec_fast_multi_jobs_kernel<1, true>),
                     reinterpret_cast<const void *>(ldpc_dec_fast_multi_jobs_kernel<4, false>), reinterpret_cast<const void *>(ldpc_dec_fast_multi_jobs_kernel<4, true>)};
  for (size_t i = 0; i < sizeof(k) / sizeof(k[0]); i++) {
    const hipError_t e = hipFuncSetAttribute(k[i], hipFuncAttributeMaxDynamicSharedMemorySize, 160 * 1024);
    if (e != hipSuccess)
      return e;
  }
  return hipSuccess;
}

hipError_t ldpc_launch_dec_fast(const ldpc_dec_args &a0, const ldpc_code_desc_t &hc, uint32_t n_blocks, hipStream_t stream)
{
  if (n_blocks == 0)
    return hipSuccess;
  if (a0.jobs)
    return ldpc_launch_dec_fast_jobs(a0, hc.f_n_threads, hc.f_lds_total, n_blocks, stream);
  ldpc_dec_args a = a0;
  ldpc_fill_llr_extents(a, hc);
  a.n_blocks = n_blocks;
  if (ldpc_fast_zc_enabled(hc.Z) && hc.f_mb == 1 && hc.f_rstride == hc.Z + 4 && hc.f_astride == 2 * hc.Z && !a.trace) {
    if (a.use_crc ? ldpc_launch_zc<false, true>(hc.Z, n_blocks, hc.f_n_threads, hc.f_lds_total, stream, a)
                  : ldpc_launch_zc<false, false>(hc.Z, n_blocks, hc.f_n_threads, hc.f_lds_total, stream, a))
      return hipGetLastError();
  }
  if (a.use_crc)
    hipLaunchKernelGGL((ldpc_dec_fast_kernel<false, true>), dim3(n_blocks), dim3(hc.f_n_threads), hc.f_lds_total, stream, a);
  else if (a.trace)
    hipLaunchKernelGGL((ldpc_dec_fast_kernel<false, false, true>), dim3(n_blocks), dim3(hc.f_n_threads), hc.f_lds_total, stream, a);
  else
    hipLaunchKernelGGL((ldpc_dec_fast_kernel<false, false>), dim3(n_blocks), dim3(hc.f_n_threads), hc.f_lds_total, stream, a);
  return hipGetLastError();
}

hipError_t ldpc_launch_dec_fast_multi(const ldpc_dec_args &a0, const ldpc_code_desc_t &hc, uint32_t n_blocks, hipStream_t stream)
{
  if (n_blocks == 0)
    return hipSuccess;
  if (a0.jobs || !hc.f_ok || (hc.f_sub != 4 && hc.f_mb < 2))
    return hipErrorInvalidValue;
  ldpc_dec_args a = a0;
  a.n_blocks = n_blocks;
  const uint32_t per_wg = (uint32_t)hc.f_mb * (uint32_t)hc.f_sub;
  const dim3 grid((n_blocks + per_wg - 1) / per_wg), block(hc.f_n_threads);
  if (hc.f_sub == 4) {
    if (a.use_crc)
      hipLaunchKernelGGL((ldpc_dec_fast_multi_kernel<4, true>), grid, block, hc.f_lds_total, stream, a);
    else
      hipLaunchKernelGGL((ldpc_dec_fast_multi_kernel<4, false>), grid, block, hc.f_lds_total, stream, a);
  } else {
    if (a.use_crc)
      hipLaunchKernelGGL((ldpc_dec_fast_multi_kernel<1, true>), grid, block, hc.f_lds_total, stream, a);
    else
      hipLaunchKernelGGL((ldpc_dec_fast_multi_kernel<1, false>), grid, block, hc.f_lds_total, stream, a);
  }
  return hipGetLastError();
}

hipError_t ldpc_launch_dec_fast_multi_jobs(const ldpc_dec_args &a, int sub, int n_threads, int lds_bytes, uint32_t n_groups,
                                           hipStream_t stream)
{
  if (n_groups == 0)
    return hipSuccess;
  if (!a.jobs || !a.mgroups)
    return hipErrorInvalidValue;
  if (sub == 4) {
    if (a.use_crc)
      hipLaunchKernelGGL((ldpc_dec_fast_multi_jobs_kernel<4, true>), dim3(n_groups), dim3(n_threads), lds_bytes, stream, a);
    else
      hipLaunchKernelGGL((ldpc_dec_fast_multi_jobs_kernel<4, false>), dim3(n_groups), dim3(n_threads), lds_bytes, stream, a);
  } else {
    if (a.use_crc)
      hipLaunchKernelGGL((ldpc_dec_fast_multi_jobs_kernel<1, true>), dim3(n_groups), dim3(n_threads), lds_bytes, stream, a);
    else
      hipLaunchKernelGGL((ldpc_dec_fast_multi_jobs_kernel<1, false>), dim3(n_groups), dim3(n_threads), lds_bytes, stream, a);
  }
  return hipGetLastError();
}

hipError_t ldpc_launch_dec_fast_pull(const ldpc_dec_args &a0, const ldpc_code_desc_t &hc, uint32_t n_blocks, hipStream_t stream)
{
  if (n_blocks == 0)
    return hipSuccess;
  if (a0.jobs || !a0.pull)
    return hipErrorInvalidValue;
  ldpc_dec_args a = a0;
  ldpc_fill_llr_extents(a, hc);
  a.warm_ahead = 0;
  if (a.use_crc)
    hipLaunchKernelGGL(ldpc_dec_fast_pull_kernel<true>, dim3(n_blocks), dim3(hc.f_n_threads), hc.f_lds_total, stream, a);
  else
    hipLaunchKernelGGL(ldpc_dec_fast_pull_kernel<false>, dim3(n_blocks), dim3(hc.f_n_threads), hc.f_lds_total, stream, a);
  return hipGetLastError();
}

hipError_t ldpc_launch_dec_fast_jobs(const ldpc_dec_args &a, int n_threads, int lds_bytes, uint32_t n_blocks, hipStream_t stream, int zc)
{
  if (n_blocks == 0)
    return hipSuccess;
  if (ldpc_fast_zc_enabled(zc)) {
    if (a.use_crc ? ldpc_launch_zc<true, true>(zc, n_blocks, n_threads, lds_bytes, stream, a)
                  : ldpc_launch_zc<true, false>(zc, n_blocks, n_threads, lds_bytes, stream, a))
      return hipGetLastError();
  }
  if (a.use_crc)
    hipLaunchKernelGGL((ldpc_dec_fast_kernel<true, true>), dim3(n_blocks), dim3(n_threads), lds_bytes, stream, a);
  else
    hipLaunchKernelGGL((ldpc_dec_fast_kernel<true, false>), dim3(n_blocks), dim3(n_threads), lds_bytes, stream, a);
  return hipGetLastError();
}
```

openairinterface5g_amd/csrc/ldpc_server.hip:

```cpp
#include <hip/hip_runtime.h>
#include "ldpc_server.h"
#include "ldpc_dec_fast_block.h"
#include "ldpc_dec_generic_block.h"
#include "ldpc_enc_packed_core.h"

#ifndef SRV_THREADS
#define SRV_THREADS 1024
#endif
#define SRV_ENC_GROUP 128

__device__ __forceinline__ uint32_t srv_ld_sys(const uint32_t *p)
{
  return __hip_atomic_load(p, __ATOMIC_RELAXED, __HIP_MEMORY_SCOPE_SYSTEM);
}
__device__ __forceinline__ void srv_st_sys(uint32_t *p, uint32_t v)
{
  __hip_atomic_store(p, v, __ATOMIC_RELAXED, __HIP_MEMORY_SCOPE_SYSTEM);
}

typedef uint32_t srv_u32x4 __attribute__((ext_vector_type(4)));
__device__ __forceinline__ void srv_st16_sys(void *p, uint32_t a, uint32_t b, uint32_t c, uint32_t d)
{
  const srv_u32x4 v = {a, b, c, d};
  asm volatile("global_store_dwordx4 %0, %1, off sc0 sc1\n\ts_nop 1" : : "v"(p), "v"(v) : "memory");
}

typedef const srv_args LDPC_CONST_AS *srv_args_ptr_t;

template <typename T> __device__ __forceinline__ T *srv_sgpr(T *p)
{
  const uint64_t v = reinterpret_cast<uint64_t>(p);
  return reinterpret_cast<T *>(((uint64_t)(uint32_t)LDPC_UNIFORM((uint32_t)(v >> 32)) << 32) | (uint64_t)(uint32_t)LDPC_UNIFORM((uint32_t)v));
}

template <bool CRC> struct srv_fast_io {
  const srv_req *rq;
  const uint8_t *host_llr;
  const uint8_t *staged;
  uint8_t *hout;
  srv_args_ptr_t a;
  uint32_t *st;
  int tid_;
  bool resident_;
  uint32_t tag_;
  __device__ __forceinline__ const uint32_t *src32() const { return reinterpret_cast<const uint32_t *>(staged); }
  __device__ __forceinline__ const uint32_t *src32_prologue() const { return reinterpret_cast<const uint32_t *>(host_llr); }
  __device__ __forceinline__ uint32_t *stage_core() const { return reinterpret_cast<uint32_t *>(const_cast<uint8_t *>(staged)); }
  __device__ __forceinline__ int8_t *out() const { return reinterpret_cast<int8_t *>(hout); }
  __device__ __forceinline__ int max_pass() const { return LDPC_UNIFORM((int)rq->max_pass); }
  __device__ __forceinline__ int use_crc() const { return CRC ? 1 : 0; }
  __device__ __forceinline__ int crcE() const { return LDPC_UNIFORM((int)rq->crcE); }
  __device__ __forceinline__ const uint32_t *crc_pow() const { return a->crc_pow_tbl[LDPC_UNIFORM(rq->kind_mode >> 24) & 3u]; }
  __device__ __forceinline__ int out_mode() const { return LDPC_UNIFORM((int)((rq->kind_mode >> 8) & 0xffu)); }
  __device__ __forceinline__ int *tb_abort() const { return nullptr; }
  const uint32_t *abw_;
  __device__ __forceinline__ uint32_t abort_load() const
  {
    return __hip_atomic_load((const __attribute__((address_space(1))) uint32_t *)abw_, __ATOMIC_RELAXED, __HIP_MEMORY_SCOPE_SYSTEM);
  }
  __device__ __forceinline__ bool abort_is(uint32_t w) const { return w == tag_; }
  __device__ __forceinline__ bool has_abort() const { return true; }
  __device__ __forceinline__ uint32_t *stamps() const { return st; }
  static constexpr bool pass_stamps = false;
  __device__ __forceinline__ int fair_turns() const { return 0; }
  __device__ __forceinline__ int tid() const { return tid_; }
  __device__ __forceinline__ bool eager_check() const { return true; }
  static constexpr bool mute_items = false;
  __device__ __forceinline__ bool mute_check() const { return false; }
  static constexpr bool bn_tickets = false;
  static constexpr bool tb_epilogue = false;
  static constexpr bool syndrome = !CRC;
  __device__ __forceinline__ bool tables_resident() const { return resident_; }
  __device__ __forceinline__ int n_app(ldpc_code_ptr_t code, int zq) const { return ldpc_desc_n_app(code, zq); }
  __device__ __forceinline__ int n_ext(ldpc_code_ptr_t code, int zq) const { return ldpc_desc_n_ext(code, zq); }
  static constexpr bool warm_next = false;
  __device__ __forceinline__ uint32_t out_tag() const { return tag_; }
  __device__ __forceinline__ void put16(uint4 *p, uint32_t x, uint32_t y, uint32_t z, uint32_t t) const { srv_st16_sys(p, x, y, z, t); }
  __device__ __forceinline__ uint32_t ld_llr(const uint32_t *p) const { return srv_ld_sys(p); }
};

template <bool ENC = false>
__global__ void __launch_bounds__(SRV_THREADS) ldpc_server_kernel(const srv_args args_by_value)
{
  extern __shared__ __attribute__((aligned(16))) uint8_t fsm[];
  uint32_t *bc = reinterpret_cast<uint32_t *>(fsm + SRV_BC_OFF);
  uint32_t hdr = 4;
#define SRV_ARGS() ({ uint64_t p_ = args_u64; asm volatile("" : "+s"(p_)); (srv_args_ptr_t)p_; })
  (void)args_by_value;
  const uint64_t args_u64 = (uint64_t)__builtin_amdgcn_kernarg_segment_ptr();
  srv_args_ptr_t a = SRV_ARGS();
#define SRV_SLOT() (blockIdx.x)
  if (threadIdx.x == 0) {
    srv_slot_ctl *slot = a->ctl + SRV_SLOT();
    bc[20] = bc[21] = 0;
    bc[1] = srv_ld_sys(&slot->done);
    if (blockIdx.x == 0) {
      atomicMax(&a->gctl->last_activity, (long long)wall_clock64());
      srv_st_sys(a->state, 2u * a->gen + 1u);
    }
  }
  for (;;) {
    a = SRV_ARGS();
    if (threadIdx.x < 64) {
      const uint32_t *line = reinterpret_cast<const uint32_t *>(a->req + SRV_SLOT());
      const uint32_t last = bc[1], gen = a->gen;
      const int w = blockIdx.x, lane = threadIdx.x;
      uint32_t d, word = 0;
      for (;;) {
        if (lane < 16)
          word = srv_ld_sys(line + lane);
        const uint32_t hs = (w == 0 && lane == 0) ? srv_ld_sys(a->host_stop) : 0u;
        const uint32_t t0 = __builtin_amdgcn_readlane(word, 0), t1 = __builtin_amdgcn_readlane(word, 4),
                       t2 = __builtin_amdgcn_readlane(word, 8), t3 = __builtin_amdgcn_readlane(word, 12);
        d = t0;
        if (t0 != last && t0 == t1 && t0 == t2 && t0 == t3)
          break;
        if (__hip_atomic_load(&a->gctl->stopping_gen, __ATOMIC_RELAXED, __HIP_MEMORY_SCOPE_AGENT) == gen) {
          d = 0xffffffffu;
          break;
        }
        if (w == 0) {
          const long long idle = (long long)wall_clock64() -
                                 __hip_atomic_load(&a->gctl->last_activity, __ATOMIC_RELAXED, __HIP_MEMORY_SCOPE_AGENT);
          if ((uint32_t)__builtin_amdgcn_readfirstlane(hs) == gen || idle > (long long)a->idle_ticks) {
            __hip_atomic_store(&a->gctl->stopping_gen, gen, __ATOMIC_RELAXED, __HIP_MEMORY_SCOPE_AGENT);
            d = 0xffffffffu;
            break;
          }
        }
        __builtin_amdgcn_s_sleep(2);
      }
      if (lane < 16)
        bc[hdr + lane] = word;
      if (lane == 0) {
        bc[0] = d;
        bc[2] = (uint32_t)wall_clock64();
      }
    }
    __syncthreads();
    const uint32_t d = bc[0];
    if (d == 0xffffffffu)
      break;
    a = SRV_ARGS();
    if (threadIdx.x == 0)
      bc[3] = (uint32_t)wall_clock64();
    const srv_req *rq = reinterpret_cast<const srv_req *>(bc + hdr);
    hdr ^= 4u ^ 32u;
    const uint32_t kind = LDPC_UNIFORM(rq->kind_mode) & 0xffu;
    ldpc_code_ptr_t code = (ldpc_code_ptr_t)(((uint64_t)(uint32_t)LDPC_UNIFORM(rq->code_hi) << 32) | (uint64_t)(uint32_t)LDPC_UNIFORM(rq->code_lo));
    const uint8_t *host_in = srv_sgpr(a->in_host + (size_t)SRV_SLOT() * SRV_IN_STRIDE);
    uint8_t *hout = srv_sgpr(a->out_host + (size_t)SRV_SLOT() * SRV_OUT_STRIDE);
    int n_iter = 0;
    if (!ENC && kind == SRV_KIND_DEC_FAST) {
      int tid_l = (int)threadIdx.x;
      const uint8_t *staged = srv_sgpr(a->staging + (size_t)blockIdx.x * SRV_IN_STRIDE);
      const bool resident = bc[20] == LDPC_UNIFORM(rq->code_lo) && bc[21] == LDPC_UNIFORM(rq->code_hi);
      const uint32_t *abw = srv_sgpr(a->abort_w + 16u * SRV_SLOT());
      if (LDPC_UNIFORM((int)((rq->kind_mode >> 16) & 0xffu))) {
        const srv_fast_io<true> io{rq, host_in, staged, hout, a, bc + 24, tid_l, resident, d, abw};
        n_iter = ldpc_dec_fast_block(fsm, code, io);
      } else {
        const srv_fast_io<false> io{rq, host_in, staged, hout, a, bc + 24, tid_l, resident, d, abw};
        n_iter = ldpc_dec_fast_block(fsm, code, io);
      }
      if (threadIdx.x == 0) {
        bc[20] = rq->code_lo;
        bc[21] = rq->code_hi;
      }
    } else if (!ENC && kind == SRV_KIND_DEC_GENERIC) {
      __atomic_thread_fence(__ATOMIC_ACQUIRE);
      if (threadIdx.x == 0)
        bc[20] = bc[21] = 0;
      ldpc_gblock_io io;
      io.llr = reinterpret_cast<const int8_t *>(host_in);
      io.out = reinterpret_cast<int8_t *>(hout);
      io.max_pass = LDPC_UNIFORM((int)rq->max_pass);
      io.use_crc = LDPC_UNIFORM((int)((rq->kind_mode >> 16) & 0xffu));
      io.crcE = LDPC_UNIFORM((int)rq->crcE);
      io.crc_pow = a->crc_pow_tbl[LDPC_UNIFORM(rq->kind_mode >> 24) & 3u];
      io.out_mode = LDPC_UNIFORM((int)((rq->kind_mode >> 8) & 0xffu));
      io.tb_abort = nullptr;
      io.trace = nullptr;
      io.trace_stride = 0;
      n_iter = ldpc_dec_generic_block(reinterpret_cast<int8_t *>(fsm), code, io);
    } else if (ENC && kind == SRV_KIND_ENC) {
      __atomic_thread_fence(__ATOMIC_ACQUIRE);
      const int tid = threadIdx.x, grp = tid / SRV_ENC_GROUP, gt = tid - grp * SRV_ENC_GROUP;
      const int n_seg = LDPC_UNIFORM((int)(rq->kb_nseg >> 16)), Kb = LDPC_UNIFORM((int)(rq->kb_nseg & 0xffffu));
      const int words = ldpc_encp_lds_words(code->ncols, code->kb_full, code->Z, code->nrows, code->nedges);
      ldpc_encp_lds L;
      ldpc_encp_carve(reinterpret_cast<uint32_t *>(fsm) + (size_t)grp * ((words + 3) & ~3), code, L);
      const uint8_t *in = host_in + (size_t)grp * LDPC_UNIFORM(rq->seg_in_stride);
      uint8_t *out = hout + (size_t)grp * LDPC_UNIFORM(rq->seg_out_stride);
      for (int ph = 0; ph < LDPC_ENCP_NUM_PHASES; ph++) {
        if (grp < n_seg)
          ldpc_encp_phase(ph, code, Kb, in, L, out, gt, SRV_ENC_GROUP);
        __syncthreads();
      }
    }
    const uint32_t t_decoded = (uint32_t)wall_clock64();
    uint32_t sd = 0, pp = 0;
    if (threadIdx.x == 0) {
      const uint32_t clip = 0xffffu;
      const uint32_t dt_stage = bc[3] - bc[2], dt_dec = t_decoded - bc[3];
      const uint32_t dt_pro = kind == SRV_KIND_DEC_FAST ? bc[24] - bc[3] : 0u, dt_pas = kind == SRV_KIND_DEC_FAST ? bc[25] - bc[24] : 0u;
      sd = (dt_stage < clip ? dt_stage : clip) | ((dt_dec < clip ? dt_dec : clip) << 16);
      pp = (dt_pro < clip ? dt_pro : clip) | ((dt_pas < clip ? dt_pas : clip) << 16);
    }
    if (kind == SRV_KIND_DEC_FAST) {
      if (threadIdx.x == 0) {
        srv_slot_ctl *slot = a->ctl + SRV_SLOT();
        srv_st16_sys(slot, d, (uint32_t)n_iter, sd, pp);
      }
    } else {
      if (threadIdx.x == 0) {
        srv_slot_ctl *slot = a->ctl + SRV_SLOT();
        srv_st_sys(reinterpret_cast<uint32_t *>(&slot->n_iter), (uint32_t)n_iter);
        srv_st_sys(&slot->t_stage_decode, sd);
        srv_st_sys(&slot->t_pro_passes, pp);
      }
      __builtin_amdgcn_fence(__ATOMIC_RELEASE, "");
      __syncthreads();
      a = SRV_ARGS();
      if (threadIdx.x == 0) {
        srv_slot_ctl *slot = a->ctl + SRV_SLOT();
        __hip_atomic_store(&slot->done, d, __ATOMIC_RELEASE, __HIP_MEMORY_SCOPE_SYSTEM);
      }
    }
    if (threadIdx.x == 0) {
      atomicMax(&a->gctl->last_activity, (long long)wall_clock64());
      bc[1] = d;
    }
  }
  a = SRV_ARGS();
  if (threadIdx.x == 0 && blockIdx.x == 0)
    srv_st_sys(a->state, 2u * a->gen + 2u);
#undef SRV_ARGS
#undef SRV_SLOT
}

int ldpc_server_has_encoder(void) { return 1; }

hipError_t ldpc_server_init(void)
{
  const hipError_t e = hipFuncSetAttribute(reinterpret_cast<const void *>(ldpc_server_kernel<false>), hipFuncAttributeMaxDynamicSharedMemorySize,
                                           SRV_LDS_BYTES);
  if (e != hipSuccess)
    return e;
  return hipFuncSetAttribute(reinterpret_cast<const void *>(ldpc_server_kernel<true>), hipFuncAttributeMaxDynamicSharedMemorySize, SRV_LDS_BYTES);
}

hipError_t ldpc_server_launch(const srv_args &a, uint32_t n_slots, hipStream_t stream, int encoder)
{
  if (encoder)
    hipLaunchKernelGGL(ldpc_server_kernel<true>, dim3(n_slots), dim3(SRV_THREADS), SRV_LDS_BYTES, stream, a);
  else
    hipLaunchKernelGGL(ldpc_server_kernel<false>, dim3(n_slots), dim3(SRV_THREADS), SRV_LDS_BYTES, stream, a);
  return hipGetLastError();
}
```

openairinterface5g_amd/csrc/tb_rx_fused.hip:

```cpp
#include <hip/hip_runtime.h>
#include "ldpc_kernels.h"
#include "tb_chain.h"
#include "tb_rx_core.h"
#include "ldpc_dec_fast_block.h"

typedef const tb_rx_seg_job LDPC_CONST_AS *tb_seg_ptr_t;
typedef const tb_rx_tb_job LDPC_CONST_AS *tb_tb_ptr_t;

template <class T> __device__ __forceinline__ void tb_store_out(T *p, T v) { __hip_atomic_store(p, v, __ATOMIC_RELAXED, __HIP_MEMORY_SCOPE_SYSTEM); }
__device__ __forceinline__ void tb_wait_stores()
{
#if defined(__HIP_DEVICE_COMPILE__)
  asm volatile("s_waitcnt vmcnt(0)" ::: "memory");
#endif
}

template <bool LROW, bool MUTE = false> struct tb_rx_fused_io {
  const ldpc_dec_args &a;
  const tb_rx_fused_args &x;
  ldpc_job_ptr_t job;
  uint8_t *lds;
  bool tables_early = false;
  __device__ __forceinline__ tb_seg_ptr_t seg() const { return (tb_seg_ptr_t)x.segs + job->seg_idx; }
  __device__ __forceinline__ tb_tb_ptr_t tb() const { return (tb_tb_ptr_t)x.tbs + seg()->tb; }
  __device__ __forceinline__ const uint32_t *src32() const
  {
    if constexpr (LROW)
      return reinterpret_cast<const uint32_t *>(lds + x.lrow_off);
    else
      return reinterpret_cast<const uint32_t *>(a.llr + (size_t)job->llr_off);
  }
  __device__ __forceinline__ int8_t *out() const { return a.out + (size_t)job->out_off; }
  __device__ __forceinline__ int max_pass() const { return job->num_max_iter + 1; }
  __device__ __forceinline__ int use_crc() const { return 1; }
  static constexpr bool syndrome = false;
  __device__ __forceinline__ int crcE() const { return job->E; }
  __device__ __forceinline__ const uint32_t *crc_pow() const { return a.crc_pow_tbl[job->crc_type & 3]; }
  __device__ __forceinline__ int out_mode() const { return 0; }
  __device__ __forceinline__ int *tb_abort() const { return (a.tb_abort && job->abort_idx >= 0) ? a.tb_abort + job->abort_idx : nullptr; }
  __device__ __forceinline__ uint32_t *stamps() const { return nullptr; }
  static constexpr bool pass_stamps = false;
  __device__ __forceinline__ int fair_turns() const { return a.fair; }
  __device__ __forceinline__ int tid() const { return (int)threadIdx.x; }
  __device__ __forceinline__ bool eager_check() const { return false; }
  static constexpr bool mute_items = MUTE;
  __device__ __forceinline__ bool mute_check() const { return job->crc_type & LDPC_JOB_MUTE_CHECK; }
  static constexpr bool bn_tickets = true;
  __device__ __forceinline__ bool tables_resident() const { return tables_early; }
  __device__ __forceinline__ uint32_t out_tag() const { return 0u; }
  __device__ __forceinline__ uint32_t abort_load() const { return 0u; }
  __device__ __forceinline__ bool abort_is(uint32_t) const { return false; }
  __device__ __forceinline__ bool has_abort() const { return true; }
  __device__ __forceinline__ void put16(uint4 *p, uint32_t x0, uint32_t y, uint32_t z, uint32_t t) const { *p = make_uint4(x0, y, z, t); }
  __device__ __forceinline__ uint32_t ld_llr(const uint32_t *p) const { return *p; }
  __device__ __forceinline__ const uint32_t *src32_prologue() const { return src32(); }
  __device__ __forceinline__ uint32_t *stage_core() const { return nullptr; }
  __device__ __forceinline__ int n_app(ldpc_code_ptr_t code, int zq) const { return ldpc_desc_n_app(code, zq); }
  __device__ __forceinline__ int n_ext(ldpc_code_ptr_t code, int zq) const { return ldpc_desc_n_ext(code, zq); }
  static constexpr bool warm_next = false;
  static constexpr bool tb_epilogue = true;
  __device__ __forceinline__ bool tb_fused() const { return job->seg_idx >= 0; }

  template <class Bits> __device__ __forceinline__ void tb_finish(int n_iter, Bits bits_word, int *flags) const
  {
    const uint32_t tid = threadIdx.x, nt = blockDim.x, lane = tid & 63u;
    if (x.prio_pro & 2u)
      __builtin_amdgcn_s_setprio(3);
    if (x.trace && tid == 0)
      x.trace[(size_t)blockIdx.x * 16 + 4] = wall_clock64();
    const tb_seg_ptr_t sj = seg();
    const tb_tb_ptr_t tj = tb();
    const uint32_t tbi = sj->tb, C = tj->C, seg_bytes = tj->seg_bytes, bbytes = tj->B >> 3, abytes = tj->A >> 3;
    const uint32_t first = sj->r * seg_bytes;
    uint32_t count = 0;
    if (first < bbytes)
      count = first + seg_bytes <= bbytes ? seg_bytes : bbytes - first;
    const bool ok = n_iter <= (int)tj->num_max_iter;
    const uint32_t gen_prev = ((const uint32_t LDPC_CONST_AS *)x.gen)[tbi];
    uint32_t xr = 0;
    if (ok) {
      uint8_t *dst = x.payload + tj->payload_off + first;
      const uint32_t pay_n = first < abytes ? (count < abytes - first ? count : abytes - first) : 0u;
      const bool al = (reinterpret_cast<uintptr_t>(dst) & 3) == 0;
      const uint32_t Bt = tj->B - 8 * first;
      const uint32_t *pow = x.pow24a;
      for (uint32_t w = tid; 4 * w < count; w += nt) {
        uint32_t word = bits_word((int)w);
        const uint32_t nb = count - 4 * w;
        if (nb < 4)
          word &= (1u << (8 * nb)) - 1u;
        if (4 * w < pay_n) {
          const uint32_t pb = pay_n - 4 * w;
          if (pb >= 4 && al) {
            tb_store_out(reinterpret_cast<uint32_t *>(dst + 4 * w), word);
          } else {
            for (uint32_t k = 0; k < 4 && k < pb; k++)
              tb_store_out(dst + 4 * w + k, (uint8_t)(word >> (8 * k)));
          }
        }
        if (C > 1) {
#pragma unroll
          for (int q = 0; q < 8; q++) {
            const uint32_t i = 32 * w + 4 * (uint32_t)q;
            if (i < 8 * count) {
              const uint4 pw = *reinterpret_cast<const uint4 *>(pow + (Bt - 4 - i));
              const uint32_t nib = (word >> (8 * (q >> 1) + ((q & 1) ? 0 : 4))) & 0xfu;
              xr ^= (pw.w & (0u - ((nib >> 3) & 1u))) ^ (pw.z & (0u - ((nib >> 2) & 1u))) ^ (pw.y & (0u - ((nib >> 1) & 1u))) ^
                    (pw.x & (0u - (nib & 1u)));
            }
          }
        }
      }
    }
    for (int off = 32; off; off >>= 1)
      xr ^= __shfl_xor(xr, off);
    if (lane == 0 && xr)
      atomicXor(reinterpret_cast<unsigned int *>(&flags[2]), xr);
    int before = 0;
    if (tid == 0)
      before = __hip_atomic_fetch_add(&x.done[tbi], 1, __ATOMIC_RELAXED, __HIP_MEMORY_SCOPE_AGENT);
    tb_wait_stores();
    __syncthreads();
    const uint32_t gen = gen_prev + 1u;
    if (tid == 0) {
      const unsigned long long slot = (unsigned long long)(ok ? (uint32_t)flags[2] : 0u) |
                                      ((unsigned long long)(((uint32_t)n_iter & 0xffffu) | (gen << 16)) << 32);
      __hip_atomic_store(&x.slots[job->seg_idx], slot, __ATOMIC_RELAXED, __HIP_MEMORY_SCOPE_AGENT);
      if (before == (int)C - 1)
        flags[4] = 1;
    }
    __syncthreads();
    if (!flags[4])
      return;
    if (tid < 64) {
      const int nmi = (int)tj->num_max_iter;
      int imax = 0, bad = 0;
      uint32_t crc = 0;
      for (uint32_t r = lane; r < C; r += 64) {
        unsigned long long v;
        while ((uint32_t)((v = __hip_atomic_load(&x.slots[tj->seg0 + r], __ATOMIC_RELAXED, __HIP_MEMORY_SCOPE_AGENT)) >> 48) != (gen & 0xffffu))
          __builtin_amdgcn_s_sleep(2);
        const int it = (int)((v >> 32) & 0xffffu);
        imax = it > imax ? it : imax;
        bad |= it > nmi;
        crc ^= (uint32_t)v;
      }
      for (int off = 32; off; off >>= 1) {
        const int o = __shfl_xor(imax, off);
        imax = o > imax ? o : imax;
        bad |= __shfl_xor(bad, off);
        crc ^= __shfl_xor(crc, off);
      }
      if (lane == 0) {
        __hip_atomic_store(&x.done[tbi], 0, __ATOMIC_RELAXED, __HIP_MEMORY_SCOPE_AGENT);
        __hip_atomic_store(&x.gen[tbi], gen, __ATOMIC_RELAXED, __HIP_MEMORY_SCOPE_AGENT);
        if (a.tb_abort)
          __hip_atomic_store(&a.tb_abort[tbi], 0, __ATOMIC_RELAXED, __HIP_MEMORY_SCOPE_AGENT);
        const int ackv = !bad && (C == 1 || crc == 0);
        tb_store_out(x.ack + tbi, (uint8_t)ackv);
        tb_store_out(x.iter_max + tbi, imax > nmi + 1 ? nmi + 1 : imax);
        flags[5] = ackv;
      }
    }
    __syncthreads();
    if (!flags[5]) {
      uint8_t *dst = x.payload + tj->payload_off;
      const uint32_t head = (uint32_t)((4 - (reinterpret_cast<uintptr_t>(dst) & 3)) & 3);
      for (uint32_t k = tid; k < head && k < abytes; k += nt)
        tb_store_out(dst + k, (uint8_t)0);
      if (abytes > head) {
        const uint32_t nw = (abytes - head) >> 2;
        for (uint32_t w = tid; w < nw; w += nt)
          tb_store_out(reinterpret_cast<uint32_t *>(dst + head) + w, 0u);
        for (uint32_t k = head + 4 * nw + tid; k < abytes; k += nt)
          tb_store_out(dst + k, (uint8_t)0);
      }
    }
  }
};

template <bool LROW, bool MUTE, int ZC = 0, bool SCR = false, bool SYM = false>
__global__ void __launch_bounds__(1024) tb_rx_fused_kernel(const ldpc_dec_args a, const tb_rx_fused_args x)
{
  LDPC_DYNAMIC_LDS(uint8_t, fsm);
  const ldpc_job_ptr_t job = (ldpc_job_ptr_t)a.jobs + blockIdx.x;
  ldpc_code_ptr_t code = (ldpc_code_ptr_t)job->code;
  tb_rx_fused_io<LROW, MUTE> io{a, x, job, fsm};
  if (x.stagger_ticks && blockIdx.x >= x.stagger_cus && blockIdx.x < x.stagger_cus * x.stagger_slots) {
    const long long until = (long long)wall_clock64() + (long long)(blockIdx.x / x.stagger_cus) * (long long)x.stagger_ticks;
    while ((long long)wall_clock64() < until)
      __builtin_amdgcn_s_sleep(32);
  }
  unsigned long long *tr = x.trace ? x.trace + (size_t)blockIdx.x * 16 : nullptr;
  if (tr && threadIdx.x == 0) {
    tr[0] = __builtin_amdgcn_s_getreg((31 << 11) | 4);
    tr[1] = __builtin_amdgcn_s_getreg((3 << 11) | 20);
    tr[2] = wall_clock64();
  }
  if (LROW || io.tb_fused()) {
    if (x.prio_pro)
      __builtin_amdgcn_s_setprio(3);
    const tb_seg_ptr_t sj = io.seg();
    const tb_rx_geom g = tb_rx_geometry(sj);
    int8_t *l;
    if constexpr (LROW)
      l = reinterpret_cast<int8_t *>(fsm + x.lrow_off);
    else
      l = const_cast<int8_t *>(a.llr) + sj->l_off;
    if constexpr (SYM)
      tb_rx_dematch_block_sym(g, sj->Qm, x.llr + (sj->llr_off - sj->bit_off), sj->plane, x.harq + sj->harq_off, l, reinterpret_cast<int16_t *>(fsm),
                              sj->c_init, sj->bit_off, tr ? tr + 7 : nullptr);
    else if constexpr (SCR)
      tb_rx_dematch_block_scr(g, sj->Qm, x.llr + sj->llr_off, x.harq + sj->harq_off, l, reinterpret_cast<int16_t *>(fsm), sj->c_init,
                              sj->bit_off, tr ? tr + 7 : nullptr);
    else
      tb_rx_dematch_block(g, sj->Qm, x.llr + sj->llr_off, x.harq + sj->harq_off, l, reinterpret_cast<int16_t *>(fsm), tr ? tr + 7 : nullptr);
    if (2u * g.span <= (uint32_t)code->f_lds_etbl) {
      ldpc_fast_tables_to_lds(fsm, code, (int)threadIdx.x, (int)blockDim.x);
      io.tables_early = true;
    }
    if constexpr (LROW) {
      __builtin_amdgcn_fence(__ATOMIC_RELEASE, "workgroup", "local");
      __builtin_amdgcn_s_barrier();
      __builtin_amdgcn_fence(__ATOMIC_ACQUIRE, "workgroup", "local");
    } else {
      __builtin_amdgcn_fence(__ATOMIC_RELEASE, "workgroup");
      __syncthreads();
      __builtin_amdgcn_fence(__ATOMIC_ACQUIRE, "workgroup");
    }
    if (tr && threadIdx.x == 0)
      tr[10] = wall_clock64();
    if (x.prio_pro)
      __builtin_amdgcn_s_setprio(0);
  }
  if (tr && threadIdx.x == 0)
    tr[3] = wall_clock64();
  const int n_iter = ldpc_dec_fast_block<tb_rx_fused_io<LROW, MUTE>, ZC>(fsm, code, io);
  if (tr && threadIdx.x == 0) {
    tr[5] = wall_clock64();
    tr[6] = (unsigned long long)n_iter;
  }
  if (!io.tb_fused() && threadIdx.x == 0)
    a.n_iter[(uint32_t)job->iter_idx] = n_iter;
}

template <bool SCR, bool SYM = false> static hipError_t tb_rx_fused_init_t(void)
{
  const void *k[] = {reinterpret_cast<const void *>(tb_rx_fused_kernel<false, false, 0, SCR, SYM>), reinterpret_cast<const void *>(tb_rx_fused_kernel<true, false, 0, SCR, SYM>),
#define X(z) \
                     reinterpret_cast<const void *>(tb_rx_fused_kernel<false, false, z, SCR, SYM>), reinterpret_cast<const void *>(tb_rx_fused_kernel<true, false, z, SCR, SYM>), \
                     reinterpret_cast<const void *>(tb_rx_fused_kernel<false, true, z, SCR, SYM>), reinterpret_cast<const void *>(tb_rx_fused_kernel<true, true, z, SCR, SYM>),
                     LDPC_FAST_ZC_LIST(X)
#undef X
                     reinterpret_cast<const void *>(tb_rx_fused_kernel<false, true, 0, SCR, SYM>), reinterpret_cast<const void *>(tb_rx_fused_kernel<true, true, 0, SCR, SYM>)};
  for (const void *f : k) {
    const hipError_t e = hipFuncSetAttribute(f, hipFuncAttributeMaxDynamicSharedMemorySize, 160 * 1024);
    if (e != hipSuccess)
      return e;
  }
  return hipSuccess;
}
hipError_t tb_rx_fused_init(void)
{
  hipError_t e = tb_rx_fused_init_t<false>();
  if (e == hipSuccess)
    e = tb_rx_fused_init_t<true>();
  return e != hipSuccess ? e : tb_rx_fused_init_t<true, true>();
}

template <bool SCR, bool SYM = false>
static hipError_t tb_launch_rx_fused_t(const ldpc_dec_args &a, const tb_rx_fused_args &x, int n_threads, int lds_bytes, uint32_t n_jobs, hipStream_t s)
{
  if (ldpc_fast_zc_enabled((int)x.zc)) {
    switch ((int)x.zc) {
#define X(z) \
  case z: \
    if (x.lrow_off && x.mute) \
      hipLaunchKernelGGL((tb_rx_fused_kernel<true, true, z, SCR, SYM>), dim3(n_jobs), dim3(n_threads), lds_bytes, s, a, x); \
    else if (x.lrow_off) \
      hipLaunchKernelGGL((tb_rx_fused_kernel<true, false, z, SCR, SYM>), dim3(n_jobs), dim3(n_threads), lds_bytes, s, a, x); \
    else if (x.mute) \
      hipLaunchKernelGGL((tb_rx_fused_kernel<false, true, z, SCR, SYM>), dim3(n_jobs), dim3(n_threads), lds_bytes, s, a, x); \
    else \
      hipLaunchKernelGGL((tb_rx_fused_kernel<false, false, z, SCR, SYM>), dim3(n_jobs), dim3(n_threads), lds_bytes, s, a, x); \
    return hipGetLastError();
      LDPC_FAST_ZC_LIST(X)
#undef X
      default:
        break;
    }
  }
  if (x.lrow_off && x.mute)
    hipLaunchKernelGGL((tb_rx_fused_kernel<true, true, 0, SCR, SYM>), dim3(n_jobs), dim3(n_threads), lds_bytes, s, a, x);
  else if (x.lrow_off)
    hipLaunchKernelGGL((tb_rx_fused_kernel<true, false, 0, SCR, SYM>), dim3(n_jobs), dim3(n_threads), lds_bytes, s, a, x);
  else if (x.mute)
    hipLaunchKernelGGL((tb_rx_fused_kernel<false, true, 0, SCR, SYM>), dim3(n_jobs), dim3(n_threads), lds_bytes, s, a, x);
  else
    hipLaunchKernelGGL((tb_rx_fused_kernel<false, false, 0, SCR, SYM>), dim3(n_jobs), dim3(n_threads), lds_bytes, s, a, x);
  return hipGetLastError();
}

hipError_t tb_launch_rx_fused(const ldpc_dec_args &a, const tb_rx_fused_args &x, int n_threads, int lds_bytes, uint32_t n_jobs, hipStream_t s)
{
  if (n_jobs == 0)
    return hipSuccess;
  if (!a.jobs || !x.segs || !x.tbs)
    return hipErrorInvalidValue;
  if (x.scr && x.sym)
    return tb_launch_rx_fused_t<true, true>(a, x, n_threads, lds_bytes, n_jobs, s);
  return x.scr ? tb_launch_rx_fused_t<true>(a, x, n_threads, lds_bytes, n_jobs, s) : tb_launch_rx_fused_t<false>(a, x, n_threads, lds_bytes, n_jobs, s);
}
```

Before: 80.21.

## Batch check-node edge loads ahead of arithmetic to keep more LDS reads in flight

Splits the per-edge check-node work into a load phase and an arithmetic phase, and adds a sweep helper that issues up to FL edge loads (table entry, LLR words, message word) before consuming them. An empty asm memory fence and register pins stop the compiler from interleaving the loads back into the arithmetic. The window alignbyte is now done on raw registers instead of inside a combined load. Flight depth is 8 for the ps/ps2 paths and 0 for the deg-19 paths by default, enabled for all IO types through a new cn_flight flag. This trades higher VGPR pressure, with possible occupancy loss, for better latency hiding of LDS and global reads.

```diff
diff --git a/openairinterface5g_amd/csrc/ldpc_dec_fast_block.h b/openairinterface5g_amd/csrc/ldpc_dec_fast_block.h
--- a/openairinterface5g_amd/csrc/ldpc_dec_fast_block.h
+++ b/openairinterface5g_amd/csrc/ldpc_dec_fast_block.h
@@ -322,15 +322,15 @@
               ldpc_fast_item_zero_messages(L, e0b, deg, jb, Z, rstride);
             }
           } else if (p == 1)
-            (void)ldpc_fast_cn2_dispatch<true, false>(deg, L, e0a, ja, e0b, jb, Z, rstride, mb);
+            (void)ldpc_fast_cn2_dispatch<true, false, IO::cn_flight>(deg, L, e0a, ja, e0b, jb, Z, rstride, mb);
           else if (with_syn) {
             if constexpr (IO::syndrome) {
-              const uint32_t ma = ldpc_fast_cn2_dispatch<false, true>(deg, L, e0a, ja, e0b, jb, Z, rstride, mb);
+              const uint32_t ma = ldpc_fast_cn2_dispatch<false, true, IO::cn_flight>(deg, L, e0a, ja, e0b, jb, Z, rstride, mb);
               const int valida = (int)(reca >> 16) - 4 * ja, validb = (int)(recb >> 16) - 4 * jb;
               tsyn = (ma & ldpc_fast_valid_lanes(valida)) | (mb & ldpc_fast_valid_lanes(validb));
             }
           } else
-            (void)ldpc_fast_cn2_dispatch<false, false>(deg, L, e0a, ja, e0b, jb, Z, rstride, mb);
+            (void)ldpc_fast_cn2_dispatch<false, false, IO::cn_flight>(deg, L, e0a, ja, e0b, jb, Z, rstride, mb);
         }
       } else if (item < gend) {
         const bool pair = deg == 19 && code->f_pair19;
@@ -352,29 +352,29 @@
         } else if (p == 1) {
 #if defined(__HIP_DEVICE_COMPILE__)
           if (pair)
-            (void)ldpc_fast_cn19_pair<true, false>(L, e0, j, Z, rstride, half);
+            (void)ldpc_fast_cn19_pair<true, false, IO::cn_flight ? LDPC_CN_FLIGHT_P19 : 0>(L, e0, j, Z, rstride, half);
           else
 #endif
-            (void)ldpc_fast_cn_dispatch<true, false>(deg, ext, L, e0, j, Z, rstride);
+            (void)ldpc_fast_cn_dispatch<true, false, IO::cn_flight>(deg, ext, L, e0, j, Z, rstride);
         } else if (with_syn) {
           if constexpr (IO::syndrome) {
             uint32_t m;
 #if defined(__HIP_DEVICE_COMPILE__)
             if (pair)
-              m = ldpc_fast_cn19_pair<false, true>(L, e0, j, Z, rstride, half);
+              m = ldpc_fast_cn19_pair<false, true, IO::cn_flight ? LDPC_CN_FLIGHT_P19 : 0>(L, e0, j, Z, rstride, half);
             else
 #endif
-              m = ldpc_fast_cn_dispatch<false, true>(deg, ext, L, e0, j, Z, rstride);
+              m = ldpc_fast_cn_dispatch<false, true, IO::cn_flight>(deg, ext, L, e0, j, Z, rstride);
             const int valid = (int)(rowrec >> 16) - 4 * j;
             tsyn = m & ldpc_fast_valid_lanes(valid);
           }
         } else {
 #if defined(__HIP_DEVICE_COMPILE__)
           if (pair)
-            (void)ldpc_fast_cn19_pair<false, false>(L, e0, j, Z, rstride, half);
+            (void)ldpc_fast_cn19_pair<false, false, IO::cn_flight ? LDPC_CN_FLIGHT_P19 : 0>(L, e0, j, Z, rstride, half);
           else
 #endif
-            (void)ldpc_fast_cn_dispatch<false, false>(deg, ext, L, e0, j, Z, rstride);
+            (void)ldpc_fast_cn_dispatch<false, false, IO::cn_flight>(deg, ext, L, e0, j, Z, rstride);
         }
       }
       LDPC_TLOG_END(0, deg);
diff --git a/openairinterface5g_amd/csrc/ldpc_dec_fast_core.h b/openairinterface5g_amd/csrc/ldpc_dec_fast_core.h
--- a/openairinterface5g_amd/csrc/ldpc_dec_fast_core.h
+++ b/openairinterface5g_amd/csrc/ldpc_dec_fast_core.h
@@ -134,35 +134,123 @@
 #endif
 }
 
+#ifdef LDPC_CN_FLIGHT
+#define LDPC_CN_FLIGHT_DFL(n) (LDPC_CN_FLIGHT)
+#else
+#define LDPC_CN_FLIGHT_DFL(n) (n)
+#endif
+#ifndef LDPC_CN_FLIGHT_PS
+#define LDPC_CN_FLIGHT_PS LDPC_CN_FLIGHT_DFL(8)
+#endif
+#ifndef LDPC_CN_FLIGHT_PS2
+#define LDPC_CN_FLIGHT_PS2 LDPC_CN_FLIGHT_DFL(8)
+#endif
+#ifndef LDPC_CN_FLIGHT_P19
+#define LDPC_CN_FLIGHT_P19 LDPC_CN_FLIGHT_DFL(0)
+#endif
+#ifndef LDPC_CN_FLIGHT_TM
+#define LDPC_CN_FLIGHT_TM LDPC_CN_FLIGHT_DFL(0)
+#endif
+#ifndef LDPC_CN_PIN
+#define LDPC_CN_PIN 1
+#endif
+LDPC_HD void ldpc_cn_fence()
+{
+#if defined(__HIP_DEVICE_COMPILE__)
+  asm volatile("" ::: "memory");
+#endif
+}
+LDPC_HD void ldpc_cn_pin(uint32_t &a)
+{
+#if defined(__HIP_DEVICE_COMPILE__)
+  asm volatile("" : "+v"(a));
+#endif
+}
+LDPC_HD void ldpc_cn_pin(uint32_t &a, uint32_t &b)
+{
+#if defined(__HIP_DEVICE_COMPILE__)
+  asm volatile("" : "+v"(a), "+v"(b));
+#endif
+}
+template <int D, int FL, class ENTRY, class LOAD, class PIN, class USE>
+LDPC_HD void ldpc_cn_sweep(ENTRY entry, LOAD load, PIN pin, USE use)
+{
+  constexpr int C = FL <= 0 ? 1 : (FL < D ? FL : D);
+  uint32_t info[D];
+  if (FL > 0) {
+#pragma unroll
+    for (int k = 0; k < D; k++)
+      info[k] = entry(k);
+  }
+#pragma unroll
+  for (int k0 = 0; k0 < D; k0 += C) {
+#pragma unroll
+    for (int k = k0; k < k0 + C && k < D; k++)
+      load(k, FL > 0 ? info[k] : entry(k));
+    if (FL > 0)
+      ldpc_cn_fence();
+#pragma unroll
+    for (int k = k0; k < k0 + C && k < D; k++) {
+      if (FL > 0 && LDPC_CN_PIN)
+        pin(k);
+      use(k);
+    }
+  }
+}
+struct ldpc_cn_raw { uint32_t lo, hi, sh, rw; };
+template <bool IS_EXT>
+LDPC_HD void ldpc_fast_cn_edge_pin(ldpc_cn_raw &w, bool has_rw)
+{
+  if (IS_EXT)
+    ldpc_cn_pin(w.lo);
+  else
+    ldpc_cn_pin(w.lo, w.hi);
+  if (has_rw)
+    ldpc_cn_pin(w.rw);
+}
+template <bool IS_EXT>
+LDPC_HD ldpc_cn_raw ldpc_fast_cn_edge_load(const ldpc_fast_lds &L, uint32_t info, int t, const uint8_t *rp, bool want_rw)
+{
+  ldpc_cn_raw w;
+  w.rw = want_rw ? *reinterpret_cast<const uint32_t *>(rp) : 0u;
+  if (IS_EXT) {
+    w.lo = L.ext_global ? *reinterpret_cast<const uint32_t *>(L.gllr + info + (uint32_t)t) : ldpc_lds_ld32(L.base, info + (uint32_t)t);
+    w.hi = w.sh = 0u;
+  } else {
+    w.sh = info + (uint32_t)t;
+    w.lo = ldpc_lds_ld32(L.base, w.sh & ~3u);
+    w.hi = ldpc_lds_ld32(L.base, (w.sh & ~3u) + 4u);
+  }
+  return w;
+}
 template <bool IS_EXT, bool P1 = false>
-LDPC_HD void ldpc_fast_cn_edge(const ldpc_fast_lds &L, uint32_t info, int t, uint32_t rw, bool first, uint32_t &de, uint32_t &dod,
-                               uint32_t &parw, uint32_t &exte, uint32_t &exto)
+LDPC_HD void ldpc_fast_cn_edge_arith(const ldpc_fast_lds &L, const ldpc_cn_raw &w, bool first, uint32_t &de, uint32_t &dod, uint32_t &parw,
+                                     uint32_t &exte, uint32_t &exto)
 {
   if (IS_EXT) {
-    const uint32_t lw = L.ext_global ? (*reinterpret_cast<const uint32_t *>(L.gllr + info + (uint32_t)t) ^ 0x80808080u)
-                                     : ldpc_lds_ld32(L.base, info + (uint32_t)t);
+    const uint32_t lw = L.ext_global ? (w.lo ^ 0x80808080u) : w.lo;
     const uint32_t ae = ldpc_unpack_even(lw), ao = ldpc_unpack_odd(lw);
     if (first) {
-      exte = ae + (P1 ? 0x00800080u : ldpc_unpack_even(rw));
-      exto = ao + (P1 ? 0x00800080u : ldpc_unpack_odd(rw));
+      exte = ae + (P1 ? 0x00800080u : ldpc_unpack_even(w.rw));
+      exto = ao + (P1 ? 0x00800080u : ldpc_unpack_odd(w.rw));
     }
     de = ldpc_psub_sm(ae, 0x00800080u);
     dod = ldpc_psub_sm(ao, 0x00800080u);
   } else {
-    const uint32_t aw = ldpc_window(L.base, info + (uint32_t)t);
+    const uint32_t aw = ldpc_alignbyte(w.hi, w.lo, w.sh);
     if (first)
       parw ^= aw;
     if (P1) {
       de = ldpc_psub_sm(ldpc_unpack_even(aw), 0x00800080u);
       dod = ldpc_psub_sm(ldpc_unpack_odd(aw), 0x00800080u);
     } else {
-      de = ldpc_psub_sm(ldpc_unpack_even(aw), ldpc_unpack_even(rw));
-      dod = ldpc_psub_sm(ldpc_unpack_odd(aw), ldpc_unpack_odd(rw));
-    }
-  }
-}
-
-template <int D, bool EXT, int MODE, bool P1 = false, bool SYN = true>
+      de = ldpc_psub_sm(ldpc_unpack_even(aw), ldpc_unpack_even(w.rw));
+      dod = ldpc_psub_sm(ldpc_unpack_odd(aw), ldpc_unpack_odd(w.rw));
+    }
+  }
+}
+
+template <int D, bool EXT, int MODE, bool P1 = false, bool SYN = true, int FL = LDPC_CN_FLIGHT_TM>
 LDPC_HD uint32_t ldpc_fast_cn(const ldpc_fast_lds &L, int e0, int j, int Z, int rstride, int boff_r = 0, int boff_a = 0)
 {
   const int t = 4 * j + boff_r, ta = 4 * j + boff_a;
@@ -172,15 +260,25 @@
   uint32_t sxl = 0, sxh = 0, parw = 0, extl = 0, exth = 0;
   uint8_t *rrow = L.r + e0 * rstride + t;
   uint8_t *rpad = rrow + (j == 0 ? Z : 0);
-#pragma unroll
-  for (int k = 0; k < D; k++) {
-    const uint32_t info = L.etbl[e0 + k];
-    const uint32_t rw = (P1 || (!SYN && EXT && k == D - 1)) ? 0u : *reinterpret_cast<const uint32_t *>(rrow + k * rstride);
+  ldpc_cn_raw raw[D];
+  auto entry = [&](int k) { return L.etbl[e0 + k]; };
+  auto load1 = [&](int k, uint32_t info) {
+    const bool want_rw = !(P1 || (!SYN && EXT && k == D - 1));
+    raw[k] = (EXT && k == D - 1) ? ldpc_fast_cn_edge_load<true>(L, info, t, rrow + k * rstride, want_rw)
+                                 : ldpc_fast_cn_edge_load<false>(L, info, ta, rrow + k * rstride, want_rw);
+  };
+  auto pin1 = [&](int k) {
+    if (EXT && k == D - 1)
+      ldpc_fast_cn_edge_pin<true>(raw[k], !(P1 || !SYN));
+    else
+      ldpc_fast_cn_edge_pin<false>(raw[k], !P1);
+  };
+  ldpc_cn_sweep<D, FL>(entry, load1, pin1, [&](int k) {
     uint32_t dl, dh;
     if (EXT && k == D - 1)
-      ldpc_fast_cn_edge<true, P1>(L, info, t, rw, SYN, dl, dh, parw, extl, exth);
+      ldpc_fast_cn_edge_arith<true, P1>(L, raw[k], SYN, dl, dh, parw, extl, exth);
     else
-      ldpc_fast_cn_edge<false, P1>(L, info, ta, rw, SYN, dl, dh, parw, extl, exth);
+      ldpc_fast_cn_edge_arith<false, P1>(L, raw[k], SYN, dl, dh, parw, extl, exth);
     if (MODE <= 1) {
       d_lo[k] = dl;
       d_hi[k] = dh;
@@ -197,26 +295,13 @@
     m1l = ldpc_pminu(m1l, ml);
     m2h = ldpc_pminu(m2h, ldpc_pmaxu(m1h, mh));
     m1h = ldpc_pminu(m1h, mh);
-  }
+  });
   const ldpc_v2u cap = ldpc_splatu(0x8000 + 127);
   m1l = ldpc_pminu(m1l, cap); m2l = ldpc_pminu(m2l, cap);
   m1h = ldpc_pminu(m1h, cap); m2h = ldpc_pminu(m2h, cap);
   const uint32_t sl = (ldpc_u2u32(m1l) - 0x80008000u) + ldpc_u2u32(m2l), sh = (ldpc_u2u32(m1h) - 0x80008000u) + ldpc_u2u32(m2h);
   const uint32_t sx4 = ldpc_perm(sxh, sxl, LDPC_SEL_SIGNS) ^ 0x80808080u;
-#pragma unroll
-  for (int k = 0; k < D; k++) {
-    uint32_t dl, dh;
-    if (MODE <= 1) {
-      dl = d_lo[k];
-      dh = d_hi[k];
-    } else {
-      const uint32_t info = L.etbl[e0 + k];
-      const uint32_t rw = (P1 || (EXT && k == D - 1)) ? 0u : *reinterpret_cast<const uint32_t *>(rrow + k * rstride);
-      if (EXT && k == D - 1)
-        ldpc_fast_cn_edge<true, P1>(L, info, t, rw, false, dl, dh, parw, extl, exth);
-      else
-        ldpc_fast_cn_edge<false, P1>(L, info, ta, rw, false, dl, dh, parw, extl, exth);
-    }
+  auto put = [&](int k, uint32_t dl, uint32_t dh) {
     const ldpc_v2u ml = KEEP ? ldpc_as_v2u(g_lo[k]) : ldpc_sm_key(dl);
     const ldpc_v2u mh = KEEP ? ldpc_as_v2u(g_hi[k]) : ldpc_sm_key(dh);
     const uint32_t ol = sl - ldpc_u2u32(ldpc_pminu(ml, m2l)), oh = sh - ldpc_u2u32(ldpc_pminu(mh, m2h));
@@ -224,11 +309,36 @@
     const uint32_t w = ldpc_fast_cn_out_bytes(o4, sx4, ldpc_perm(dh, dl, LDPC_SEL_SIGNS));
     *reinterpret_cast<uint32_t *>(rrow + k * rstride) = w;
     *reinterpret_cast<uint32_t *>(rpad + k * rstride) = w;
+  };
+  if (MODE <= 1) {
+#pragma unroll
+    for (int k = 0; k < D; k++)
+      put(k, d_lo[k], d_hi[k]);
+  } else {
+    auto load2 = [&](int k, uint32_t info) {
+      const bool want_rw = !(P1 || (EXT && k == D - 1));
+      raw[k] = (EXT && k == D - 1) ? ldpc_fast_cn_edge_load<true>(L, info, t, rrow + k * rstride, want_rw)
+                                   : ldpc_fast_cn_edge_load<false>(L, info, ta, rrow + k * rstride, want_rw);
+    };
+    auto pin2 = [&](int k) {
+      if (EXT && k == D - 1)
+        ldpc_fast_cn_edge_pin<true>(raw[k], false);
+      else
+        ldpc_fast_cn_edge_pin<false>(raw[k], !P1);
+    };
+    ldpc_cn_sweep<D, FL>(entry, load2, pin2, [&](int k) {
+      uint32_t dl, dh;
+      if (EXT && k == D - 1)
+        ldpc_fast_cn_edge_arith<true, P1>(L, raw[k], false, dl, dh, parw, extl, exth);
+      else
+        ldpc_fast_cn_edge_arith<false, P1>(L, raw[k], false, dl, dh, parw, extl, exth);
+      put(k, dl, dh);
+    });
   }
   return SYN ? ldpc_fast_odd_lanes<LDPC_SEL_EO>(parw, EXT, extl, exth, D) : 0u;
 }
 
-template <int D, bool EXT, bool P1 = false, bool SYN = true>
+template <int D, bool EXT, bool P1 = false, bool SYN = true, int FL = LDPC_CN_FLIGHT_PS>
 LDPC_HD uint32_t ldpc_fast_cn_ps(const ldpc_fast_lds &L, int e0, int j, int Z, int rstride, int boff_r = 0, int boff_a = 0)
 {
   const int t = 4 * j + boff_r, ta = 4 * j + boff_a;
@@ -238,15 +348,25 @@
   uint32_t sx4 = 0, parw = 0, extl = 0, exth = 0;
   uint8_t *rrow = L.r + e0 * rstride + t;
   uint8_t *rpad = rrow + (j == 0 ? Z : 0);
-#pragma unroll
-  for (int k = 0; k < D; k++) {
-    const uint32_t info = L.etbl[e0 + k];
-    const uint32_t rw = (P1 || (!SYN && EXT && k == D - 1)) ? 0u : *reinterpret_cast<const uint32_t *>(rrow + k * rstride);
+  ldpc_cn_raw raw[D];
+  auto entry = [&](int k) { return L.etbl[e0 + k]; };
+  auto load = [&](int k, uint32_t info) {
+    const bool want_rw = !(P1 || (!SYN && EXT && k == D - 1));
+    raw[k] = (EXT && k == D - 1) ? ldpc_fast_cn_edge_load<true>(L, info, t, rrow + k * rstride, want_rw)
+                                 : ldpc_fast_cn_edge_load<false>(L, info, ta, rrow + k * rstride, want_rw);
+  };
+  auto pin = [&](int k) {
+    if (EXT && k == D - 1)
+      ldpc_fast_cn_edge_pin<true>(raw[k], !(P1 || !SYN));
+    else
+      ldpc_fast_cn_edge_pin<false>(raw[k], !P1);
+  };
+  ldpc_cn_sweep<D, FL>(entry, load, pin, [&](int k) {
     uint32_t dl, dh;
     if (EXT && k == D - 1)
-      ldpc_fast_cn_edge<true, P1>(L, info, t, rw, SYN, dl, dh, parw, extl, exth);
+      ldpc_fast_cn_edge_arith<true, P1>(L, raw[k], SYN, dl, dh, parw, extl, exth);
     else
-      ldpc_fast_cn_edge<false, P1>(L, info, ta, rw, SYN, dl, dh, parw, extl, exth);
+      ldpc_fast_cn_edge_arith<false, P1>(L, raw[k], SYN, dl, dh, parw, extl, exth);
     const ldpc_v2u ml = ldpc_sm_key(dl);
     const ldpc_v2u mh = ldpc_sm_key(dh);
     m_lo[k] = ldpc_u2u32(ml);
@@ -258,7 +378,7 @@
       p_lo[i] = ldpc_u2u32(ldpc_pmin3_keys(i ? ldpc_as_v2u(p_lo[i - 1]) : cap, ldpc_as_v2u(m_lo[k - 1]), ml));
       p_hi[i] = ldpc_u2u32(ldpc_pmin3_keys(i ? ldpc_as_v2u(p_hi[i - 1]) : cap, ldpc_as_v2u(m_hi[k - 1]), mh));
     }
-  }
+  });
   sx4 ^= 0x80808080u;
   auto put = [&](int k, ldpc_v2u ol, ldpc_v2u oh) {
     const uint32_t o4 = ldpc_perm(ldpc_u2u32(oh), ldpc_u2u32(ol), 0x06020400u);
@@ -288,7 +408,7 @@
   return SYN ? ldpc_fast_odd_lanes<LDPC_SEL_EO>(parw, EXT, extl, exth, D) : 0u;
 }
 
-template <int D, bool EXT, bool P1 = false, bool SYN = true>
+template <int D, bool EXT, bool P1 = false, bool SYN = true, int FL = LDPC_CN_FLIGHT_PS2>
 LDPC_HD uint32_t ldpc_fast_cn_ps2(const ldpc_fast_lds &L, int e0a, int ja, int e0b, int jb, int Z, int rstride, uint32_t &mask_b)
 {
   constexpr int N = 2, NP = D / 2;
@@ -302,21 +422,38 @@
     rrow[n] = L.r + e0[n] * rstride + t[n];
     rpad[n] = rrow[n] + (t[n] == 0 ? Z : 0);
   }
-#pragma unroll
-  for (int k = 0; k < D; k++) {
-    uint32_t info[N], rw[N];
+  ldpc_cn_raw raw[N][D];
+  uint32_t info_b[D];
+  auto entry = [&](int k) {
+    info_b[k] = L.etbl[e0[1] + k];
+    return L.etbl[e0[0] + k];
+  };
+  auto load = [&](int k, uint32_t info_a) {
+    const bool want_rw = !(P1 || (!SYN && EXT && k == D - 1));
 #pragma unroll
     for (int n = 0; n < N; n++) {
-      info[n] = L.etbl[e0[n] + k];
-      rw[n] = (P1 || (!SYN && EXT && k == D - 1)) ? 0u : *reinterpret_cast<const uint32_t *>(rrow[n] + k * rstride);
-    }
+      const uint32_t info = n ? info_b[k] : info_a;
+      raw[n][k] = (EXT && k == D - 1) ? ldpc_fast_cn_edge_load<true>(L, info, t[n], rrow[n] + k * rstride, want_rw)
+                                      : ldpc_fast_cn_edge_load<false>(L, info, t[n], rrow[n] + k * rstride, want_rw);
+    }
+  };
+  auto pin = [&](int k) {
+#pragma unroll
+    for (int n = 0; n < N; n++) {
+      if (EXT && k == D - 1)
+        ldpc_fast_cn_edge_pin<true>(raw[n][k], !(P1 || !SYN));
+      else
+        ldpc_fast_cn_edge_pin<false>(raw[n][k], !P1);
+    }
+  };
+  ldpc_cn_sweep<D, FL>(entry, load, pin, [&](int k) {
 #pragma unroll
     for (int n = 0; n < N; n++) {
       uint32_t dl, dh;
       if (EXT && k == D - 1)
-        ldpc_fast_cn_edge<true, P1>(L, info[n], t[n], rw[n], SYN, dl, dh, parw[n], extl[n], exth[n]);
+        ldpc_fast_cn_edge_arith<true, P1>(L, raw[n][k], SYN, dl, dh, parw[n], extl[n], exth[n]);
       else
-        ldpc_fast_cn_edge<false, P1>(L, info[n], t[n], rw[n], SYN, dl, dh, parw[n], extl[n], exth[n]);
+        ldpc_fast_cn_edge_arith<false, P1>(L, raw[n][k], SYN, dl, dh, parw[n], extl[n], exth[n]);
       const ldpc_v2u ml = ldpc_sm_key(dl);
       const ldpc_v2u mh = ldpc_sm_key(dh);
       m_lo[n][k] = ldpc_u2u32(ml);
@@ -329,7 +466,7 @@
         p_hi[n][i] = ldpc_u2u32(ldpc_pmin3_keys(i ? ldpc_as_v2u(p_hi[n][i - 1]) : cap, ldpc_as_v2u(m_hi[n][k - 1]), mh));
       }
     }
-  }
+  });
   sx4[0] ^= 0x80808080u;
   sx4[1] ^= 0x80808080u;
   auto put = [&](int n, int k, ldpc_v2u ol, ldpc_v2u oh) {
@@ -376,19 +513,19 @@
 #else
 #define LDPC_CN2_ATTR LDPC_HD
 #endif
-template <bool P1 = false, bool SYN = true>
+template <bool P1 = false, bool SYN = true, bool FLT = true>
 LDPC_CN2_ATTR uint32_t ldpc_fast_cn2_dispatch(int deg, const ldpc_fast_lds &L, int e0a, int ja, int e0b, int jb, int Z, int rstride, uint32_t &mask_b)
 {
   switch (deg) {
-    case 3: return ldpc_fast_cn_ps2<3, true, P1, SYN>(L, e0a, ja, e0b, jb, Z, rstride, mask_b);
-    case 4: return ldpc_fast_cn_ps2<4, true, P1, SYN>(L, e0a, ja, e0b, jb, Z, rstride, mask_b);
-    default: return ldpc_fast_cn_ps2<5, true, P1, SYN>(L, e0a, ja, e0b, jb, Z, rstride, mask_b);
+    case 3: return ldpc_fast_cn_ps2<3, true, P1, SYN, FLT ? LDPC_CN_FLIGHT_PS2 : 0>(L, e0a, ja, e0b, jb, Z, rstride, mask_b);
+    case 4: return ldpc_fast_cn_ps2<4, true, P1, SYN, FLT ? LDPC_CN_FLIGHT_PS2 : 0>(L, e0a, ja, e0b, jb, Z, rstride, mask_b);
+    default: return ldpc_fast_cn_ps2<5, true, P1, SYN, FLT ? LDPC_CN_FLIGHT_PS2 : 0>(L, e0a, ja, e0b, jb, Z, rstride, mask_b);
   }
 }
 
 #if defined(__HIP_DEVICE_COMPILE__)
 __device__ __forceinline__ uint32_t ldpc_swap_pair(uint32_t v) { return (uint32_t)__builtin_amdgcn_update_dpp(0, (int)v, 0xB1 , 0xf, 0xf, false); }
-template <bool P1, bool SYN = true>
+template <bool P1, bool SYN = true, int FL = LDPC_CN_FLIGHT_P19>
 __device__ __forceinline__ uint32_t ldpc_fast_cn19_pair(const ldpc_fast_lds &L, int e0, int j, int Z, int rstride, int half)
 {
   constexpr int N = 10, NP = N / 2;
@@ -399,14 +536,15 @@
   uint32_t sx4 = 0, parw = 0, extl = 0, exth = 0;
   uint8_t *rrow = L.r + ebase * rstride + t;
   uint8_t *rpad = rrow + (j == 0 ? Z : 0);
-#pragma unroll
-  for (int k = 0; k < N; k++) {
+  ldpc_cn_raw raw[N];
+  auto slot = [&](int k) { return (k < N - 1 || !half) ? k : N - 2; };
+  auto entry = [&](int k) { return L.etbl[ebase + slot(k)]; };
+  auto load = [&](int k, uint32_t info) { raw[k] = ldpc_fast_cn_edge_load<false>(L, info, t, rrow + slot(k) * rstride, !P1); };
+  auto pin = [&](int k) { ldpc_fast_cn_edge_pin<false>(raw[k], !P1); };
+  ldpc_cn_sweep<N, FL>(entry, load, pin, [&](int k) {
     const bool live = k < N - 1 || !half;
-    const int kk = live ? k : N - 2;
-    const uint32_t info = L.etbl[ebase + kk];
-    const uint32_t rw = P1 ? 0u : *reinterpret_cast<const uint32_t *>(rrow + kk * rstride);
     uint32_t dl, dh, pw = 0;
-    ldpc_fast_cn_edge<false, P1>(L, info, t, rw, SYN, dl, dh, pw, extl, exth);
+    ldpc_fast_cn_edge_arith<false, P1>(L, raw[k], SYN, dl, dh, pw, extl, exth);
     ldpc_v2u ml = ldpc_sm_key(dl);
     ldpc_v2u mh = ldpc_sm_key(dh);
     uint32_t sg = ldpc_perm(dh, dl, LDPC_SEL_SIGNS);
@@ -425,7 +563,7 @@
       p_lo[i] = ldpc_u2u32(ldpc_pmin3_keys(i ? ldpc_as_v2u(p_lo[i - 1]) : cap, ldpc_as_v2u(m_lo[k - 1]), ml));
       p_hi[i] = ldpc_u2u32(ldpc_pmin3_keys(i ? ldpc_as_v2u(p_hi[i - 1]) : cap, ldpc_as_v2u(m_hi[k - 1]), mh));
     }
-  }
+  });
   ldpc_v2u sl = ldpc_as_v2u(ldpc_swap_pair(p_lo[NP - 1])), sh = ldpc_as_v2u(ldpc_swap_pair(p_hi[NP - 1]));
   sx4 ^= ldpc_swap_pair(sx4);
   if (SYN)
@@ -492,26 +630,26 @@
 #ifndef LDPC_F_MODE_D19
 #define LDPC_F_MODE_D19 2
 #endif
-template <bool P1 = false, bool SYN = true>
+template <bool P1 = false, bool SYN = true, bool FLT = true>
 LDPC_HD uint32_t ldpc_fast_cn_dispatch(int deg, int ext, const ldpc_fast_lds &L, int e0, int j, int Z, int rstride, int boff_r = 0,
                                        int boff_a = 0)
 {
   if (!ext) {
     switch (deg) {
-      case 19: return ldpc_fast_cn<19, false, LDPC_F_MODE_D19, P1, SYN>(L, e0, j, Z, rstride, boff_r, boff_a);
-      case 10: return ldpc_fast_cn_ps<10, false, P1, SYN>(L, e0, j, Z, rstride, boff_r, boff_a);
-      default: return ldpc_fast_cn_ps<8, false, P1, SYN>(L, e0, j, Z, rstride, boff_r, boff_a);
+      case 19: return ldpc_fast_cn<19, false, LDPC_F_MODE_D19, P1, SYN, FLT ? LDPC_CN_FLIGHT_TM : 0>(L, e0, j, Z, rstride, boff_r, boff_a);
+      case 10: return ldpc_fast_cn_ps<10, false, P1, SYN, FLT ? LDPC_CN_FLIGHT_PS : 0>(L, e0, j, Z, rstride, boff_r, boff_a);
+      default: return ldpc_fast_cn_ps<8, false, P1, SYN, FLT ? LDPC_CN_FLIGHT_PS : 0>(L, e0, j, Z, rstride, boff_r, boff_a);
     }
   }
   switch (deg) {
-    case 3: return ldpc_fast_cn_ps<3, true, P1, SYN>(L, e0, j, Z, rstride, boff_r, boff_a);
-    case 4: return ldpc_fast_cn_ps<4, true, P1, SYN>(L, e0, j, Z, rstride, boff_r, boff_a);
-    case 5: return ldpc_fast_cn_ps<5, true, P1, SYN>(L, e0, j, Z, rstride, boff_r, boff_a);
-    case 6: return ldpc_fast_cn_ps<6, true, P1, SYN>(L, e0, j, Z, rstride, boff_r, boff_a);
-    case 7: return ldpc_fast_cn_ps<7, true, P1, SYN>(L, e0, j, Z, rstride, boff_r, boff_a);
-    case 8: return ldpc_fast_cn_ps<8, true, P1, SYN>(L, e0, j, Z, rstride, boff_r, boff_a);
-    case 9: return ldpc_fast_cn_ps<9, true, P1, SYN>(L, e0, j, Z, rstride, boff_r, boff_a);
-    default: return ldpc_fast_cn_ps<10, true, P1, SYN>(L, e0, j, Z, rstride, boff_r, boff_a);
+    case 3: return ldpc_fast_cn_ps<3, true, P1, SYN, FLT ? LDPC_CN_FLIGHT_PS : 0>(L, e0, j, Z, rstride, boff_r, boff_a);
+    case 4: return ldpc_fast_cn_ps<4, true, P1, SYN, FLT ? LDPC_CN_FLIGHT_PS : 0>(L, e0, j, Z, rstride, boff_r, boff_a);
+    case 5: return ldpc_fast_cn_ps<5, true, P1, SYN, FLT ? LDPC_CN_FLIGHT_PS : 0>(L, e0, j, Z, rstride, boff_r, boff_a);
+    case 6: return ldpc_fast_cn_ps<6, true, P1, SYN, FLT ? LDPC_CN_FLIGHT_PS : 0>(L, e0, j, Z, rstride, boff_r, boff_a);
+    case 7: return ldpc_fast_cn_ps<7, true, P1, SYN, FLT ? LDPC_CN_FLIGHT_PS : 0>(L, e0, j, Z, rstride, boff_r, boff_a);
+    case 8: return ldpc_fast_cn_ps<8, true, P1, SYN, FLT ? LDPC_CN_FLIGHT_PS : 0>(L, e0, j, Z, rstride, boff_r, boff_a);
+    case 9: return ldpc_fast_cn_ps<9, true, P1, SYN, FLT ? LDPC_CN_FLIGHT_PS : 0>(L, e0, j, Z, rstride, boff_r, boff_a);
+    default: return ldpc_fast_cn_ps<10, true, P1, SYN, FLT ? LDPC_CN_FLIGHT_PS : 0>(L, e0, j, Z, rstride, boff_r, boff_a);
   }
 }
 
diff --git a/openairinterface5g_amd/csrc/ldpc_decoder_fast.hip b/openairinterface5g_amd/csrc/ldpc_decoder_fast.hip
--- a/openairinterface5g_amd/csrc/ldpc_decoder_fast.hip
+++ b/openairinterface5g_amd/csrc/ldpc_decoder_fast.hip
@@ -33,6 +33,7 @@
   static constexpr bool mute_items = false;
   __device__ __forceinline__ bool mute_check() const { return false; }
   static constexpr bool bn_tickets = true;
+  static constexpr bool cn_flight = true;
   static constexpr bool tb_epilogue = false;
   __device__ __forceinline__ bool tables_resident() const { return false; }
   __device__ __forceinline__ uint32_t out_tag() const { return 0u; }
diff --git a/openairinterface5g_amd/csrc/ldpc_server.hip b/openairinterface5g_amd/csrc/ldpc_server.hip
--- a/openairinterface5g_amd/csrc/ldpc_server.hip
+++ b/openairinterface5g_amd/csrc/ldpc_server.hip
@@ -68,6 +68,7 @@
   static constexpr bool mute_items = false;
   __device__ __forceinline__ bool mute_check() const { return false; }
   static constexpr bool bn_tickets = false;
+  static constexpr bool cn_flight = true;
   static constexpr bool tb_epilogue = false;
   static constexpr bool syndrome = !CRC;
   __device__ __forceinline__ bool tables_resident() const { return resident_; }
diff --git a/openairinterface5g_amd/csrc/tb_rx_fused.hip b/openairinterface5g_amd/csrc/tb_rx_fused.hip
--- a/openairinterface5g_amd/csrc/tb_rx_fused.hip
+++ b/openairinterface5g_amd/csrc/tb_rx_fused.hip
@@ -46,6 +46,7 @@
   static constexpr bool mute_items = MUTE;
   __device__ __forceinline__ bool mute_check() const { return job->crc_type & LDPC_JOB_MUTE_CHECK; }
   static constexpr bool bn_tickets = true;
+  static constexpr bool cn_flight = true;
   __device__ __forceinline__ bool tables_resident() const { return tables_early; }
   __device__ __forceinline__ uint32_t out_tag() const { return 0u; }
   __device__ __forceinline__ uint32_t abort_load() const { return 0u; }
```

Result: no change. 81.01, median of 6 (+1.0%).
